# HerreraKrachTeichmann/NJODE

Measured on AMD Instinct MI355X. Metric: paths/sec (training step) on 20k Black-Scholes, 100 steps, higher is better.
Workload: dtype f32; 1 GPU; BlackScholes 20000 paths/GPU x 100 grid steps, every rank's paths as one batch, hidden_size=10, 3x(50,50) tanh nets, dropout 0.1, train step = plan+fwd+bwd+Adam; global_batch=20000, n_obs_rows=199470, euler_steps_per_batch=1820212, params=10071, parallelism=dp1

## Files before the change

include/njode_selftest.h:

```cpp
#ifndef NJODE_SELFTEST_H
#define NJODE_SELFTEST_H

#include <stdint.h>

#include "njode_hip.h"

#ifdef __cplusplus
extern "C" {
#endif

int njode_selftest_dropout_words(uint64_t seed, uint64_t path_id, uint32_t time_key, uint32_t net,
                                 int32_t n_words, uint32_t* out_words, void* stream);

int njode_debug_plan_stamps(unsigned long long* out, int cap_blocks);

typedef struct NjodePlanView {
  int64_t plan_bytes;
  int64_t sched;
  int64_t t_of_row, first_row, last_row;
  int64_t item_prev, item_next, item_kbeg, item_len;
  int64_t order, t_order;
  int64_t len_hist, base_s, base16_s, path_sorted, row_by_path, first_j;
  int64_t jlo, tile_base;
  int32_t n_tiles;
  int32_t generic;
  int32_t seg;
  int32_t sort_linked;
  int32_t links_only;
  int32_t tails;
  int32_t one_launch;
  int32_t plan_first_stage;
  int32_t plan_blocks;
  int32_t cs_shift, cs_nwb;
  int32_t cs_large;
  int32_t scan_thread_per_key;
  int32_t lds_cnt;
  int32_t tail_radix;
  int32_t split_on;
  int32_t split_ns[2], split_nw[2];
  float split_r[2];
} NjodePlanView;
int njode_debug_plan_view(const NjodeDims* dims, int32_t batch_size, int32_t n_obs, int32_t n_times,
                          int32_t n_steps, int32_t call_flags, NjodePlanView* out);

#ifdef __cplusplus
}
#endif
#endif
```

njode_amd/_lib.py:

```python
import ctypes as C
import os

import torch

_HERE = os.path.dirname(os.path.abspath(__file__))
LIB_PATH = os.environ.get('NJODE_LIB') or os.path.join(_HERE, 'libnjode_hip.so')

NJODE_OK = 0
E_UNSUPPORTED, E_BADARG, E_WORKSPACE, E_HIP = 1, 2, 3, 4
ACT_TANH, ACT_RELU = 0, 1
F_MASKED, F_INPUT_CURRENT_T, F_RESIDUAL, F_LOSS_EASY, F_USE_RNN = 0x1, 0x2, 0x4, 0x8, 0x10
C_TRAIN, C_GET_LOSS, C_RETURN_PATH, C_SAVE_BWD, C_LOSS_IN_BWD = 0x1, 0x2, 0x4, 0x8, 0x10
C_SCHED_KNOWN, C_SCHED_TAIL = 0x20, 0x40
C_PLAN_READY, C_NEED_HT = 0x80, 0x100
C_ROWS_IN_FWD = 0x400
C_GEN_LOCKSTEP = 0x200
C_PLAN_DEFER = 0x800

EXPORTS = ('njode_supported', 'njode_param_count', 'njode_workspace_bytes',
           'njode_plan_bytes', 'njode_plan_f32', 'njode_plan_flush', 'njode_plan_barrier_failures',
           'njode_forward_f32', 'njode_backward_f32', 'njode_backward_loss_f32',
           'njode_adam_step_f32',
           'njode_last_error', 'njode_build_info', 'njode_profile_enable',
           'njode_profile_read',
           'njode_philox4x32_10', 'njode_generate_paths', 'njode_sample_observations',
           'njode_collate_count', 'njode_collate_fill',
           'njode_cond_exp_bytes', 'njode_cond_exp_f64',
           'njode_generate_stage', 'njode_cond_exp_staged_bytes', 'njode_cond_exp_staged_f64',
           'njode_protocol_bytes', 'njode_protocol_rows', 'njode_protocol_score_f32',
           'njode_records_bytes', 'njode_records_count', 'njode_records_fill',
           'njode_records_heldout', 'njode_records_val_bytes', 'njode_records_val_count',
           'njode_records_val_fill',
           'njode_online_supported', 'njode_online_reset_f32', 'njode_online_advance_f32',
           'njode_online_observe_f32', 'njode_online_predict_f32', 'njode_online_run_f32',
           'njode_online_gen_supported', 'njode_online_tables_bytes', 'njode_online_tables_f32',
           'njode_online_gen_reset_f32', 'njode_online_gen_advance_f32', 'njode_online_gen_observe_f32',
           'njode_online_gen_predict_f32', 'njode_online_gen_run_f32',
           'njode_f64_supported', 'njode_f64_workspace_bytes', 'njode_forward_f64', 'njode_backward_f64',
           'njode_gob_supported', 'njode_gob_param_count', 'njode_gob_workspace_bytes',
           'njode_gob_forward_f32', 'njode_gob_backward_f32',
           'njode_selftest_dropout_words', 'njode_debug_plan_stamps', 'njode_debug_plan_view')
ROWS_CLOSEST, ROWS_FIRST_NEAREST = 0, 1
SDE_MODELS = {'BlackScholes': 0, 'OrnsteinUhlenbeck': 1, 'Heston': 2}
SDE_MODELS_STAGED = dict(SDE_MODELS, HestonWOFeller=3)
MAX_STAGES = 16


MAX_HIDDEN = 8


class NjodeNet(C.Structure):
    _fields_ = [('n_hidden', C.c_int32), ('width', C.c_int32 * MAX_HIDDEN),
                ('act', C.c_int32 * MAX_HIDDEN)]


class NjodeDims(C.Structure):
    _fields_ = [('input_size', C.c_int32), ('hidden_size', C.c_int32),
                ('output_size', C.c_int32), ('n_hidden', C.c_int32),
                ('width', C.c_int32), ('act', C.c_int32), ('flags', C.c_int32),
                ('per_net', C.c_int32), ('nets', NjodeNet * 3)]


class NjodeSchedule(C.Structure):
    _fields_ = [('n_steps', C.c_int32), ('n_times', C.c_int32),
                ('step_dt', C.c_void_p), ('step_t', C.c_void_p),
                ('k_jump', C.c_void_p), ('time_f32', C.c_void_p),
                ('time_ptr', C.c_void_p)]


class NjodeBatch(C.Structure):
    _fields_ = [('batch_size', C.c_int32), ('n_obs', C.c_int32),
                ('start_X', C.c_void_p), ('X', C.c_void_p), ('M', C.c_void_p),
                ('obs_idx', C.c_void_p), ('n_obs_ot', C.c_void_p),
                ('loss_batch_size', C.c_float), ('path_id_offset', C.c_int64),
                ('plan', C.c_void_p), ('grad_hT', C.c_void_p)]


class NjodeSchedule64(C.Structure):
    _fields_ = NjodeSchedule._fields_


class NjodeBatch64(C.Structure):
    _fields_ = [('batch_size', C.c_int32), ('n_obs', C.c_int32),
                ('start_X', C.c_void_p), ('X', C.c_void_p), ('M', C.c_void_p),
                ('obs_idx', C.c_void_p), ('n_obs_ot', C.c_void_p),
                ('loss_batch_size', C.c_double)]


GOB_F_BIAS, GOB_F_IMPUTE = 0x1, 0x2


class NjodeGobDims(C.Structure):
    _fields_ = [('input_size', C.c_int32), ('hidden_size', C.c_int32), ('p_hidden', C.c_int32),
                ('prep_hidden', C.c_int32), ('cov_hidden', C.c_int32), ('flags', C.c_int32)]


class NjodeSde(C.Structure):
    _fields_ = [('model', C.c_int32), ('n_paths', C.c_int32), ('dim', C.c_int32),
                ('n_steps', C.c_int32), ('has_sine', C.c_int32), ('reserved', C.c_int32),
                ('drift', C.c_double), ('volatility', C.c_double), ('mean', C.c_double),
                ('speed', C.c_double), ('correlation', C.c_double), ('S0', C.c_double),
                ('maturity', C.c_double), ('sine_coeff', C.c_double)]


class NjodeSdeStage(C.Structure):
    _fields_ = [('sde', NjodeSde), ('v0', C.c_double), ('return_vol', C.c_int32),
                ('first_step', C.c_int32)]


class NjodeCondExpSchedule(C.Structure):
    _fields_ = [('n_steps', C.c_int32), ('n_times', C.c_int32),
                ('step_dt', C.c_void_p), ('step_t', C.c_void_p),
                ('k_jump', C.c_void_p), ('time_ptr', C.c_void_p)]


class NjodeProtocolJob(C.Structure):
    _fields_ = [('pred', C.c_void_p), ('n_rows', C.c_int32), ('B', C.c_int32), ('dim', C.c_int32),
                ('n_query', C.c_int32), ('rows', C.c_void_p), ('vals', C.c_void_p),
                ('mask', C.c_void_p), ('X_val', C.c_void_p), ('M_val', C.c_void_p),
                ('index_val', C.c_void_p)]


class NjodeRecordStore(C.Structure):
    _fields_ = [('n_records', C.c_int32), ('n_rows', C.c_int32), ('dim', C.c_int32),
                ('n_grid', C.c_int32), ('drop_unobserved', C.c_int32), ('reserved', C.c_int32),
                ('row_ptr', C.c_void_p), ('row_g', C.c_void_p), ('vals', C.c_void_p),
                ('mask', C.c_void_p), ('att_min', C.c_void_p), ('att_max', C.c_void_p)]


class NjodeOnlineState(C.Structure):
    _fields_ = [('h', C.c_void_p), ('last_X', C.c_void_p), ('tau', C.c_void_p), ('now', C.c_void_p),
                ('n_series', C.c_int32)]


class NjodePlanView(C.Structure):
    OFFSETS = ('sched', 't_of_row', 'first_row', 'last_row', 'item_prev', 'item_next', 'item_kbeg',
               'item_len', 'order', 't_order', 'len_hist', 'base_s', 'base16_s', 'path_sorted',
               'row_by_path', 'first_j', 'jlo', 'tile_base')
    FLAGS = ('n_tiles', 'generic', 'seg', 'sort_linked', 'links_only', 'tails', 'one_launch',
             'plan_first_stage', 'plan_blocks', 'cs_shift', 'cs_nwb', 'cs_large', 'scan_thread_per_key', 'lds_cnt',
             'tail_radix', 'split_on')
    _fields_ = ([('plan_bytes', C.c_int64)] + [(n, C.c_int64) for n in OFFSETS]
                + [(n, C.c_int32) for n in FLAGS]
                + [('split_ns', C.c_int32 * 2), ('split_nw', C.c_int32 * 2), ('split_r', C.c_float * 2)])

    def as_dict(self):
        d = {n: int(getattr(self, n)) for n in ('plan_bytes',) + self.OFFSETS + self.FLAGS}
        d.update(split_ns=list(self.split_ns), split_nw=list(self.split_nw), split_r=list(self.split_r))
        return d


def plan_view(dims, batch_size, n_obs, n_times, n_steps, call_flags):
    v = NjodePlanView()
    check(lib().njode_debug_plan_view(C.byref(dims), batch_size, n_obs, n_times, n_steps, call_flags,
                                      C.byref(v)))
    return v.as_dict()


class NjodeError(RuntimeError):
    def __init__(self, code, msg):
        super().__init__('libnjode_hip error {}: {}'.format(code, msg))
        self.code = code


class NjodeUnsupported(NjodeError, NotImplementedError):
    pass


_lib = None


def lib():
    global _lib
    if _lib is not None:
        return _lib
    if not os.path.exists(LIB_PATH):
        raise ImportError(
            'njode_amd: {} not found. The NJ-ODE path has no CPU fallback; build '
            'the gfx950 library first: `python -m njode_amd.build` (needs hipcc).'
            .format(LIB_PATH))
    L = C.CDLL(LIB_PATH)
    vp, i32, f32, u64, sz = C.c_void_p, C.c_int32, C.c_float, C.c_uint64, C.c_size_t
    L.njode_supported.argtypes = [C.POINTER(NjodeDims)]
    L.njode_supported.restype = C.c_int
    L.njode_param_count.argtypes = [C.POINTER(NjodeDims)]
    L.njode_param_count.restype = sz
    L.njode_workspace_bytes.argtypes = [C.POINTER(NjodeDims), i32, i32, i32, i32, i32,
                                        C.POINTER(sz)]
    L.njode_workspace_bytes.restype = C.c_int
    L.njode_plan_bytes.argtypes = [C.POINTER(NjodeDims), i32, i32, i32, i32, i32, C.POINTER(sz)]
    L.njode_plan_bytes.restype = C.c_int
    L.njode_plan_f32.argtypes = [C.POINTER(NjodeDims), C.POINTER(NjodeBatch),
                                 C.POINTER(NjodeSchedule), i32, vp, sz, vp]
    L.njode_plan_f32.restype = C.c_int
# ... 150 lines not shown
```

njode_amd/csrc/njode_api.hip:

```cpp
#include <hip/hip_runtime.h>

#include <cmath>
#include <cstdio>
#include <cstring>

#include "../../include/njode_selftest.h"
#include "njode_call.h"
#include "njode_gen_host.h"
#include "njode_layout.h"

using namespace njode;

#define NJ_CFG(ID) namespace njode { const CfgOps* njode_cfg_ops_##ID(); }
#include "_generated_cfgs.inc"
#undef NJ_CFG
typedef const CfgOps* (*CfgGetter)();
static const CfgGetter g_cfgs[] = {
#define NJ_CFG(ID) njode::njode_cfg_ops_##ID,
#include "_generated_cfgs.inc"
#undef NJ_CFG
};
static const int g_ncfg = sizeof(g_cfgs) / sizeof(g_cfgs[0]);

static thread_local char g_err[512] = "";
// ... 249 lines not shown
  const size_t i = (size_t)blockIdx.x * blockDim.x + threadIdx.x;
  if (i >= n) return;
  const float pi = p[i];
  const float gi = fmaf(wd, pi, g[i] * gscale);
  const float mi = fmaf(beta1, m[i], (1.0f - beta1) * gi);
  const float vi = fmaf(beta2, v[i], (1.0f - beta2) * gi * gi);
  m[i] = mi;
  v[i] = vi;
  const float denom = sqrtf(vi) * inv_sqrt_c2 + eps;
  p[i] = pi - lr_c1 * (mi / denom);
}

TDesc transpose_desc(const CfgOps* o) {
  TDesc d;
  d.n = 0;
  const int nh = o->dims.n_hidden, W = o->dims.width, H = o->dims.hidden_size;
  const int ins[3] = {o->ode_in, o->enc_in, H};
  const int outs[3] = {H, H, o->dims.output_size};
  int off = 0;
  for (int net = 0; net < 3; ++net) {
    for (int l = 0; l <= nh; ++l) {
      const int li = l == 0 ? ins[net] : W, lo = l == nh ? outs[net] : W;
      d.l[d.n++] = {off, li, lo};
      off += li * lo + lo;
    }
  }
  if (o->dims.flags & NJODE_F_USE_RNN) {
    const int D = o->dims.input_size;
    d.l[d.n++] = {off, D, 3 * H};
    d.l[d.n++] = {off + 3 * H * D, H, 3 * H};
  }
  return d;
}

int prepare(Call& c, const NjodeDims* dims, const float* params, const NjodeBatch* b,
            const NjodeSchedule* s, int call_flags, float weight, float dropout_p,
            uint64_t seed, void* ws, size_t ws_bytes, bool want_hT, bool plan_only = false) {
  if (!dims || (!params && !plan_only) || !ws) return fail(NJODE_E_BADARG, "null argument");
  if (int rc = check_call(b, s, dims->flags, call_flags, dropout_p)) return rc;
  c.plan_only = plan_only;
  c.o = find_cfg(dims);
  if (!c.o)
    return fail(NJODE_E_UNSUPPORTED,
                "no gfx950 specialisation for d=%d H=%d d_out=%d n_hidden=%d width=%d act=%d "
                "flags=0x%x (compiled: %s)",
                dims->input_size, dims->hidden_size, dims->output_size, dims->n_hidden,
                dims->width, dims->act, dims->flags, njode_build_info());
  const int B = b->batch_size, n_obs = b->n_obs, K = s->n_steps, nt = s->n_times;
  const Sizing z = size_call(*c.o, B, n_obs, nt, K, call_flags, record_budget_bytes(), env());
  c.L = make_layout(c.o, z, B, n_obs, nt, K);
  if (ws_bytes < (plan_only ? c.L.plan_end : c.L.total))
    return fail(NJODE_E_WORKSPACE, "workspace too small: %zu < %zu", ws_bytes,
                plan_only ? c.L.plan_end : c.L.total);
  char* w = (char*)ws;
  c.planned = !plan_only && (call_flags & NJODE_C_PLAN_READY) != 0;
  if (c.planned && !b->plan) return fail(NJODE_E_BADARG, "NJODE_C_PLAN_READY without NjodeBatch.plan");
  char* pw = c.planned ? (char*)b->plan : w;
  c.pw = pw;
  KArgs& a = c.a;
  memset(&a, 0, sizeof(a));
  a.P = params;
  a.PT = (float*)(w + c.L.PT);
  a.frag = (float*)(w + c.L.frag);
  a.frag_enc = a.frag + c.o->frag_enc_off;
  a.frag_dec = a.frag + c.o->frag_dec_off;
  a.frag2 = a.frag + c.o->frag2_off;
  a.B = B;
  a.n_obs = n_obs;
  a.start_X = b->start_X;
  a.X = b->X;
  a.M = b->M;
  a.obs_idx = b->obs_idx;
  a.n_obs_ot = b->n_obs_ot;
  a.inv_batch = 1.0f / b->loss_batch_size;
  a.gid0 = (unsigned long long)b->path_id_offset;
  a.K = K;
  a.n_times = nt;
  float* sb = (float*)(pw + c.L.sched);
  a.step_dt = sb;
  a.step_t = sb + K;
  a.k_jump = (const int*)(sb + 2 * (size_t)K);
  a.time_f32 = sb + 2 * (size_t)K + nt;
  a.t_of_row = (int*)(pw + c.L.t_of_row);
  a.row_by_path = (int*)(pw + c.L.row_by_path);
  a.path_sorted = (int*)(pw + c.L.path_sorted);
  int* f3 = (int*)(pw + c.L.first3);
  a.first_j = f3;
  a.first_row = f3 + B;
  a.last_row = f3 + 2 * (size_t)B;
  int* i4 = (int*)(pw + c.L.item4);
  const size_t nr = (size_t)(n_obs > 0 ? n_obs : 1);
  a.item_prev = i4;
  a.item_next = i4 + nr;
  a.item_kbeg = i4 + 2 * nr;
  a.item_len = i4 + 3 * nr;
  a.order = (int*)(pw + c.L.order);
  a.t_order = (int*)(pw + c.L.tail4) + 3 * (size_t)B;
  a.base_s = (long long*)(pw + c.L.base_s);
  a.base16_s = (long long*)(pw + c.L.base16);
  a.act = c.L.act ? (float*)(w + c.L.act) : nullptr;
  a.dbits = c.L.dbits ? (uint32_t*)(w + c.L.dbits) : nullptr;
  a.dbits_row = c.L.dbits_row ? (uint32_t*)(w + c.L.dbits_row) : nullptr;
  a.q4_pt = z.q4_pt;
  a.chain = z.chain ? 1 : 0;
  a.h0row = (float*)(w + c.L.h0row);
  a.h0start = (float*)(w + c.L.h0start);
  a.h_end = (float*)(w + c.L.h_end);
  a.lam_end = (float*)(w + c.L.lam_end);
  a.g_h0 = (float*)(w + c.L.g_h0);
  a.lam_start = (float*)(w + c.L.lam_start);
  a.loss_terms = (float*)(w + c.L.loss_terms);
  a.traj = (float*)(w + c.L.traj);
  a.ltraj = a.traj;
  a.lam_traj = (float*)(w + c.L.lk_lam);
  a.src_row = (int*)(w + c.L.lk_src);
  float* rows = (float*)(w + c.L.lk_rows);
  const size_t nrDO = nr * dims->output_size;
  a.y_row = rows;
  a.ybj_row = rows + nrDO;
  a.g_y = rows + 2 * nrDO;
  a.g_ybj = rows + 3 * nrDO;
  a.g_hnew = rows + 4 * nrDO;
  a.g_hstart = (float*)(w + c.L.lk_hstart);
  a.lact = c.L.lk_act ? (float*)(w + c.L.lk_act) : nullptr;
  a.jact = c.L.lk_jact ? (float*)(w + c.L.lk_jact) : nullptr;
  a.cdelta = c.L.lk_delta ? (float*)(w + c.L.lk_delta) : nullptr;
  a.cseg = c.L.lk_seg ? (float*)(w + c.L.lk_seg) : nullptr;
  a.item_pack = c.L.item_pack ? (float*)(w + c.L.item_pack) : nullptr;
  a.tile_last = c.L.tile_last ? (long long*)(w + c.L.tile_last) : nullptr;
  a.slab = (float*)(w + c.L.slab);
  a.trash = (float*)(w + c.L.trash);
  a.g_hT = nullptr;
  a.n_waves = a.n_waves_ode = a.n_waves_rows = z.n_waves;
  a.weight = weight;
  a.loss_easy = (dims->flags & NJODE_F_LOSS_EASY) ? 1 : 0;
  const bool drop = (call_flags & NJODE_C_TRAIN) && dropout_p > 0.0f && dims->n_hidden > 0;
  if (drop && dims->width > 64)
    return fail(NJODE_E_UNSUPPORTED, "dropout needs width <= 64");
  const DropSetup ds = make_drop_ctx(dropout_p, seed, drop);
  a.dc = ds.dc;
  a.keep = ds.keep;
  const bool tail = (call_flags & NJODE_C_SCHED_KNOWN) ? (call_flags & NJODE_C_SCHED_TAIL) != 0
                                                        : (nt == 0 ? K > 0 : s->k_jump[nt - 1] < K);
  const Route& r = c.route = route_call(*c.o, z, B, n_obs, K, call_flags, env(), tail, drop, want_hT);
  if (!route_admitted(r))
    return fail(NJODE_E_WORKSPACE, "route not admitted by the workspace sizing (seg_chain %d / seg_items %d, "
                "lockstep kinds %d %d / chain %d lock_act %d, bits ahead %d %d / sized %d %d)",
                r.seg_chain, (int)z.seg_items, r.lock_fwd_kind, r.lock_bwd_kind, (int)z.chain, (int)z.lock_act,
                (int)r.seg_bits_ahead, (int)r.lock_bits_ahead, (int)z.seg_bits, (int)z.lock_bits);
  a.save_traj = z.save ? 1 : 0;
  a.ode_split = r.ode_split, a.seg_chain = r.seg_chain;
  a.defer_loss = r.defer_loss;
  a.n_split_blocks = r.n_split_blocks, a.n_blocks_bwd = r.n_blocks_bwd;
  a.n_split_fwd = r.n_split_fwd, a.n_blocks_fwd = r.n_blocks_fwd;
  a.dw_pair_blocks = r.dw_pair_blocks, a.dw_seg_blocks = r.dw_seg_blocks, a.dw_enc_fused = r.dw_enc_fused;
  return NJODE_OK;
}

__global__ void __launch_bounds__(1024) k_sum_small(const float* __restrict__ x, int n,
                                                    float* __restrict__ out) {
  __shared__ float sh[1024];
  float acc = 0.0f;
  for (int i = threadIdx.x; i < n; i += 1024) acc += x[i];
  sh[threadIdx.x] = acc;
  __syncthreads();
  for (int o = 512; o > 0; o >>= 1) {
    if ((int)threadIdx.x < o) sh[threadIdx.x] += sh[threadIdx.x + o];
    __syncthreads();
  }
  if (threadIdx.x == 0) out[0] = sh[0];
}
constexpr int SUM_SMALL_MAX = 16384;
void sum_to(const Call& c, void* ws, int n, float* out, hipStream_t st) {
  if (n <= SUM_SMALL_MAX) {
    k_sum_small<<<1, 1024, 0, st>>>(c.a.loss_terms, n, out);
    return;
  }
  float* partial = (float*)((char*)ws + c.L.sum_partial);
  k_sum_stage1<<<SUM_BLOCKS, 256, 0, st>>>(c.a.loss_terms, n, partial);
  k_sum_stage2<<<1, SUM_BLOCKS, 0, st>>>(partial, out);
}

int size_query(const NjodeDims* dims, int B, int n_obs, int n_times, int K, int call_flags, size_t* out, bool plan) {
  const CfgOps* o = find_cfg(dims);
  if (!o) return gen::gen_workspace_bytes(dims, B, n_obs, n_times, K, call_flags, out, plan);
  if (!out || B <= 0 || n_obs < 0 || n_times < 0 || K < 0) return fail(NJODE_E_BADARG, "bad size");
  const Layout L = make_layout(o, size_call(*o, B, n_obs, n_times, K, call_flags, record_budget_bytes(), env()),
                               B, n_obs, n_times, K);
  *out = plan ? L.plan_end : L.total;
  return NJODE_OK;
}

}

extern "C" int njode_workspace_bytes(const NjodeDims* dims, int32_t batch_size, int32_t n_obs,
                                     int32_t n_times, int32_t n_steps, int32_t call_flags, size_t* out) {
  return size_query(dims, batch_size, n_obs, n_times, n_steps, call_flags, out, false);
}

extern "C" int njode_plan_bytes(const NjodeDims* dims, int32_t batch_size, int32_t n_obs,
                                int32_t n_times, int32_t n_steps, int32_t call_flags, size_t* out) {
  return size_query(dims, batch_size, n_obs, n_times, n_steps, call_flags, out, true);
}

extern "C" int njode_debug_plan_view(const NjodeDims* dims, int32_t batch_size, int32_t n_obs, int32_t n_times,
                                     int32_t n_steps, int32_t call_flags, NjodePlanView* out) {
  if (!dims || !out) return fail(NJODE_E_BADARG, "null argument");
  memset(out, 0, sizeof(*out));
  out->sched = out->t_of_row = out->first_row = out->last_row = out->item_prev = out->item_next = out->item_kbeg =
      out->item_len = out->order = out->t_order = out->len_hist = out->base_s = out->base16_s = out->path_sorted =
          out->row_by_path = out->first_j = out->jlo = out->tile_base = -1;
  const int flags = call_flags & ~(NJODE_C_PLAN_READY | NJODE_C_PLAN_DEFER);
  size_t bytes = 0;
  if (int rc = size_query(dims, batch_size, n_obs, n_times, n_steps, flags, &bytes, true)) return rc;
  out->plan_bytes = (int64_t)bytes;
  if (!find_cfg(dims)) return gen::gen_plan_view(dims, batch_size, n_obs, n_times, n_steps, flags, out);
  alignas(256) static char anchor[256];
  NjodeBatch b{};
  b.batch_size = batch_size;
  b.n_obs = n_obs;
  b.start_X = b.X = b.M = (const float*)anchor;
  b.obs_idx = b.n_obs_ot = (const int32_t*)anchor;
  b.loss_batch_size = 1.0f;
  NjodeSchedule s{};
  s.n_steps = n_steps;
  s.n_times = n_times;
  s.step_dt = s.step_t = s.time_f32 = (const float*)anchor;
  s.k_jump = s.time_ptr = (const int32_t*)anchor;
  Call c;
  if (int rc = prepare(c, dims, nullptr, &b, &s, flags | NJODE_C_SCHED_KNOWN, 0.5f, 0.0f, 0, anchor, bytes,
                       (call_flags & NJODE_C_NEED_HT) != 0, true))
    return rc;
  const KArgs& a = c.a;
  const auto off = [&](const void* p) { return (int64_t)((const char*)p - anchor); };
  out->sched = off(a.step_dt);
  if (n_obs <= 0) return NJODE_OK;
  describe_plan(c, call_flags, out);
  out->t_of_row = off(a.t_of_row);
  out->first_row = off(a.first_row);
  out->last_row = off(a.last_row);
  out->item_prev = off(a.item_prev);
  out->item_next = off(a.item_next);
  out->item_kbeg = off(a.item_kbeg);
  out->item_len = off(a.item_len);
  out->len_hist = (int64_t)c.L.len_hist;
  if (out->sort_linked) {
    out->path_sorted = off(a.path_sorted);
    out->row_by_path = off(a.row_by_path);
    out->first_j = off(a.first_j);
  }
  if (out->seg && !out->links_only) {
    out->order = off(a.order);
    out->base_s = off(a.base_s);
    out->base16_s = off(a.base16_s);
  }
  if (out->tails) out->t_order = off(a.t_order);
  return NJODE_OK;
}

extern "C" int njode_plan_f32(const NjodeDims* dims, const NjodeBatch* batch,
                              const NjodeSchedule* sched, int32_t call_flags, void* plan,
                              size_t plan_bytes, njodeStream_t stream) {
  if (dims && !find_cfg(dims))
    return gen::gen_plan(dims, batch, sched, call_flags & ~(NJODE_C_PLAN_READY | NJODE_C_PLAN_DEFER), plan,
                         plan_bytes, (hipStream_t)stream);
  Call c;
  int rc = prepare(c, dims, nullptr, batch, sched, call_flags & ~(NJODE_C_PLAN_READY | NJODE_C_PLAN_DEFER), 0.5f,
                   0.0f, 0, plan, plan_bytes, (call_flags & NJODE_C_NEED_HT) != 0, true);
  if (rc) return rc;
  return plan_call(c, sched, call_flags, (hipStream_t)stream);
}

extern "C" int njode_forward_f32(const NjodeDims* dims, const float* params,
                                 const NjodeBatch* batch, const NjodeSchedule* sched,
                                 int32_t call_flags, float weight, float dropout_p,
                                 uint64_t seed, float* hT, float* loss, float* path_h,
                                 float* path_y, void* workspace, size_t workspace_bytes,
                                 njodeStream_t stream) {
  struct FlushGuard { ~FlushGuard() { pending_flush(); } } flush_on_any_return;
  if (dims && !find_cfg(dims)) {
    pending_flush();
    return gen::gen_forward(dims, params, batch, sched, call_flags, weight, dropout_p, seed, hT, loss,
                            path_h, path_y, workspace, workspace_bytes, (hipStream_t)stream);
  }
  Call c;
  int rc = prepare(c, dims, params, batch, sched, call_flags, weight, dropout_p, seed, workspace,
                   workspace_bytes, hT != nullptr);
  if (rc) return rc;
  const Route& r = c.route;
  hipStream_t st = (hipStream_t)stream;
  const bool want_loss = call_flags & NJODE_C_GET_LOSS, want_path = call_flags & NJODE_C_RETURN_PATH;
  if ((want_loss && !loss) || (want_path && (!path_h || !path_y)))
    return fail(NJODE_E_BADARG, "null output");
  if (!hT && !r.seg) return fail(NJODE_E_BADARG, "hT may only be omitted on the segment plan");
  if ((call_flags & NJODE_C_SAVE_BWD) && !(call_flags & NJODE_C_GET_LOSS))
    return fail(NJODE_E_BADARG, "NJODE_C_SAVE_BWD needs NJODE_C_GET_LOSS");
  c.a.hT = hT;
  c.a.path_h = path_h;
  c.a.path_y = path_y;
  if (c.planned) {
    if (r.tails && !(call_flags & NJODE_C_NEED_HT))
      return fail(NJODE_E_BADARG, "the prebuilt plan was made without NJODE_C_NEED_HT");
  } else {
    if ((rc = upload_schedule(c.pw + c.L.sched, sched, st))) return rc;
    if ((rc = build_plan(c, c.pw, st))) return rc;
  }
  PendingPlan hosted;
  pending_host_or_flush(c, st, hosted);
  if (r.seg) {
    route_side(c.route, c.a.plan_ready != nullptr);
    HIP_TRY(c.o->seg_forward(c.a, r, st));
    if (hosted.on) pending_tails(hosted);
    if (r.defer_loss != 1) sum_to(c, workspace, c.a.n_obs, loss, st);
  } else {
    HIP_TRY(c.o->lock_forward(c.a, r, st));
    if (want_loss) sum_to(c, workspace, c.a.B, loss, st);
  }
  HIP_TRY(hipGetLastError());
  return NJODE_OK;
}

static int backward_impl(const NjodeDims* dims, const float* params, const NjodeBatch* batch,
                         const NjodeSchedule* sched, int32_t call_flags, float weight,
                         float dropout_p, uint64_t seed, const float* grad_loss,
                         float* grad_params, float* loss, void* workspace,
                         size_t workspace_bytes, njodeStream_t stream) {
  if (dims && !find_cfg(dims))
    return gen::gen_backward(dims, params, batch, sched, call_flags, weight, dropout_p, seed,
                             grad_loss, grad_params, workspace, workspace_bytes, (hipStream_t)stream);
  Call c;
  int rc = prepare(c, dims, params, batch, sched, call_flags, weight, dropout_p, seed, workspace,
                   workspace_bytes, false);
  if (rc) return rc;
  const Route& r = c.route;
  if (!grad_loss || !grad_params) return fail(NJODE_E_BADARG, "null gradient pointer");
  if (!(call_flags & NJODE_C_SAVE_BWD) || !(call_flags & NJODE_C_GET_LOSS))
    return fail(NJODE_E_BADARG,
                "backward needs a forward with NJODE_C_SAVE_BWD | NJODE_C_GET_LOSS");
  hipStream_t st = (hipStream_t)stream;
  if (r.needs_PT) {
    const TDesc d = transpose_desc(c.o);
    k_transpose_params<<<cdiv(c.o->P, 256), 256, 0, st>>>(params, (float*)c.a.PT, c.o->P, d);
  }
  if (!r.seg && !r.lock_mfma && (dims->flags & NJODE_F_MASKED))
    return fail(NJODE_E_UNSUPPORTED,
                "the backward of a masked model runs on the matrix-core lockstep kernels only "
                "(2 hidden layers, width < 64, hidden_size <= 64, output_size <= 64)");
  if (r.lock_mfma) c.a.n_waves_rows = r.size.n_waves_lock;
  if (r.defer_loss == 1 && !loss)
    return fail(NJODE_E_BADARG, "NJODE_C_LOSS_IN_BWD needs njode_backward_loss_f32");
  if (batch->grad_hT && r.seg)
    return fail(NJODE_E_UNSUPPORTED, "NjodeBatch.grad_hT: the segment plan does not differentiate through hT; "
                                     "run the step with NJODE_C_GEN_LOCKSTEP");
  c.a.g_hT = batch->grad_hT;
  if (r.seg) HIP_TRY(c.o->seg_backward(c.a, r, st));
// ... 98 lines not shown
```

njode_amd/csrc/njode_cfg.hip:

```cpp
#include <type_traits>

#include "njode_route.h"
#if NJ_PART >= 4
#include "njode_chain.h"
#include "njode_chain_seg.h"
#include "njode_chain_dw.h"
#endif
#if NJ_PART == 6
#include "njode_online.h"
#endif

#define NJ_CAT_(a, b) a##b
#define NJ_CAT(a, b) NJ_CAT_(a, b)

namespace njode {

#ifndef NJ_RNN
#define NJ_RNN 0
#endif
using C = Cfg<NJ_D, NJ_H, NJ_DO, NJ_NH, NJ_W, NJ_ACT, (NJ_MASKED != 0), (NJ_CURT != 0),
              (NJ_RES != 0), (NJ_RNN != 0)>;

hipError_t NJ_CAT(njode_seg_forward_, NJ_ID)(const KArgs& a, const Route& r, hipStream_t st);
hipError_t NJ_CAT(njode_seg_backward_, NJ_ID)(const KArgs& a, const Route& r, hipStream_t st);
// ... 4 lines not shown
constexpr bool HAS_SPLIT = HAS_MFMA && SplitOk<C>::value;
constexpr bool HAS_Q4 = HAS_MFMA_SWEEP && Q4Ok<C>::value;
constexpr bool HAS_CHAIN = HAS_Q4 && ChainOk<C>::value;
void NJ_CAT(njode_chain_forward_, NJ_ID)(const KArgs& a, const Route& r, hipStream_t st);
void NJ_CAT(njode_chain_sweep_, NJ_ID)(const KArgs& a, const Route& r, hipStream_t st);
void NJ_CAT(njode_chain_dw_, NJ_ID)(const KArgs& a, hipStream_t st);
constexpr bool HAS_SEG_CHAIN = HAS_SPLIT && HAS_MFMA_SWEEP && SegChainOk<C>::value;
void NJ_CAT(njode_seg_chain_forward_, NJ_ID)(const KArgs& a, const Route& r, hipStream_t st);
void NJ_CAT(njode_seg_chain_backward_, NJ_ID)(const KArgs& a, const Route& r, hipStream_t st);

template <class F> static auto with_drop(bool drop, F f) {
  return drop ? f(std::true_type{}) : f(std::false_type{});
}
static inline const char* seg_fwd_name(const Route& r, bool tails) {
  if (r.seg_ode != ODE_MFMA) return tails ? "k_ode_fwd_items.tails" : "k_ode_fwd_items";
  if (r.seg_chain) return "k_seg_fwd_chain";
  if (r.ode_split) return tails ? "k_ode_fwd_split.tails" : "k_ode_fwd_mixed";
  return tails ? "k_ode_fwd_mfma.tails" : "k_ode_fwd_mfma";
}
static inline const char* lock_name(int kind, bool bwd) {
  if (kind == LOCK_VALU) return bwd ? "k_paths_bwd_adj" : "k_paths_fwd";
  if (kind == LOCK_CHAIN) return bwd ? "k_paths_bwd_adj_chain" : "k_paths_fwd_chain";
  return bwd ? "k_paths_bwd_adj_mfma" : "k_paths_fwd_mfma";
}
template <bool ON, class CC> struct FragSize {
  static constexpr int ode = 0, enc = 0, dec = 0;
};
template <class CC> struct FragSize<true, CC> {
  static constexpr int ode = MF<CC>::NALL * 64;
  static constexpr int enc = EncS<CC>::type::NALL * 64;
  static constexpr int dec = DecS<CC>::type::NALL * 64;
};
using FS = FragSize<(HAS_MFMA || HAS_MFMA_LOCK), C>;
constexpr int MF_FLOATS = FS::ode + FS::enc + FS::dec + FS::ode;
constexpr int FRAG2_OFF = FS::ode + FS::enc + FS::dec;
template <bool ON, class CC> struct ActSize { static constexpr int value = 0; };
template <class CC> struct ActSize<true, CC> { static constexpr int value = StepRec<CC>::PER_CHAIN; };
constexpr int ACT_FLOATS = ActSize<HAS_SPLIT, C>::value;

template <class C, class ES, class DS>
__global__ void k_pack_all(const float* __restrict__ P, float* __restrict__ frag, float* __restrict__ frag2,
                           float* __restrict__ frag_enc, float* __restrict__ frag_dec, float ik,
                           unsigned* __restrict__ zero8) {
  constexpr int N = MF<C>::NALL * 64, NE = ES::NALL * 64, ND = DS::NALL * 64;
  const int idx = blockIdx.x * blockDim.x + threadIdx.x;
  if (zero8 && idx < 8) zero8[idx] = 0;
  if (idx < N) frag[idx] = ode_frag_value<C>(P, idx, 1.0f, 1.0f);
  else if (idx < 2 * N) frag2[idx - N] = ode_frag_value<C>(P, idx - N, Ode2Scale<C>::S, ik);
  else if (idx < 2 * N + NE) pack_net_value<typename C::Enc, ES>(P + C::OFF_ENC, frag_enc, idx - 2 * N);
  else if (idx < 2 * N + NE + ND) pack_net_value<typename C::Dec, DS>(P + C::OFF_DEC, frag_dec, idx - 2 * N - NE);
}
template <class C, class ES, class DS>
__global__ void k_pack_all_bits(KArgs a, int n_pack) {
  if ((int)blockIdx.x < n_pack) {
    constexpr int N = MF<C>::NALL * 64, NE = ES::NALL * 64, ND = DS::NALL * 64;
    const int idx = blockIdx.x * blockDim.x + threadIdx.x;
    if (a.plan_sync_zero && idx < 8) a.plan_sync_zero[idx] = 0;
    if (idx < N) a.frag[idx] = ode_frag_value<C>(a.P, idx, 1.0f, 1.0f);
    else if (idx < 2 * N) a.frag2[idx - N] = ode_frag_value<C>(a.P, idx - N, Ode2Scale<C>::S, a.dc.inv_keep);
    else if (idx < 2 * N + NE) pack_net_value<typename C::Enc, ES>(a.P + C::OFF_ENC, a.frag_enc, idx - 2 * N);
    else if (idx < 2 * N + NE + ND) pack_net_value<typename C::Dec, DS>(a.P + C::OFF_DEC, a.frag_dec, idx - 2 * N - NE);
  } else {
    if constexpr (SegChainOk<C>::value) {
      if (a.seg_chain) {
        seg_chain_bits_body<C>(a, (int)blockIdx.x - n_pack, (int)gridDim.x - n_pack);
        return;
      }
    }
    if constexpr (HAS_SPLIT) {
      const int nb = (int)gridDim.x - n_pack;
      drop_bits_tile_steps<C>(a, ((int)blockIdx.x - n_pack) * 4 + (threadIdx.x >> 6), nb * 4);
    }
  }
}

template <class CC> static void launch_pack_frags(const KArgs& a, hipStream_t st, bool bits = false) {
  if constexpr (HAS_MFMA) {
    using ES = typename EncS<CC>::type;
    using DS = typename DecS<CC>::type;
    const int n_pack = cdiv((2 * MF<CC>::NALL + ES::NALL + DS::NALL) * 64, 256);
    if (bits) {
      const long long work = a.seg_chain ? (long long)a.K * a.B / 64 + 1
                                         : (long long)cdiv(a.n_obs, 16) * cdiv(a.K > 0 ? a.K : 1, 8);
      const int nb = (int)(work / 4 + 1 < 1024 ? work / 4 + 1 : 1024);
      k_pack_all_bits<CC, ES, DS><<<n_pack + nb, 256, 0, st>>>(a, n_pack);
    } else {
      k_pack_all<CC, ES, DS><<<n_pack, 256, 0, st>>>(a.P, a.frag, a.frag2, a.frag_enc, a.frag_dec, a.dc.inv_keep,
                                                  a.plan_sync_zero);
    }
  }
}
template <class CC, bool DROP> static void launch_mfma_enc(const KArgs& a, const Route& r, hipStream_t st) {
  if constexpr (HAS_MFMA) {
    const int n_tiles = cdiv(a.n_obs + a.B, 16);
    k_encode_rows_mfma<CC, DROP><<<n_tiles < r.enc_blocks ? n_tiles : r.enc_blocks, 64, 0, st>>>(a);
  }
}
template <class CC> static void lock_pack_frags(const KArgs& a, hipStream_t st) {
  if constexpr (HAS_MFMA_LOCK) {
    using ES = typename EncS<CC>::type;
    using DS = typename DecS<CC>::type;
    k_pack_frags<CC><<<cdiv(MF<CC>::NALL * 64, 256), 256, 0, st>>>(a.P, a.frag);
    k_pack_net<typename CC::Enc, ES><<<cdiv(ES::NALL * 64, 256), 256, 0, st>>>(a.P + CC::OFF_ENC,
                                                                             a.frag_enc);
    k_pack_net<typename CC::Dec, DS><<<cdiv(DS::NALL * 64, 256), 256, 0, st>>>(a.P + CC::OFF_DEC,
                                                                             a.frag_dec);
  }
}
template <class CC, bool DROP> static void launch_mfma_jump(const KArgs& a, hipStream_t st) {
  if constexpr (HAS_MFMA) {
    const int n_tiles = cdiv(a.n_obs, 16);
    k_jump_rows_mfma<CC, DROP><<<n_tiles < 2048 ? n_tiles : 2048, 64, 0, st>>>(a);
  }
}
template <class CC, bool DROP> static void launch_ode_bwd_mfma(const KArgs& a, const Route& r, hipStream_t st) {
  if constexpr (HAS_MFMA) {
    if constexpr (HAS_SPLIT) {
      if (r.ode_split) {
        ProfScope ps("k_ode_bwd_mixed", st);
        k_ode_bwd_mixed<CC, DROP><<<a.n_blocks_bwd, 256, 0, st>>>(a);
        return;
      }
    }
    ProfScope ps("k_ode_bwd_mfma", st);
    k_ode_bwd_mfma<CC, DROP><<<a.n_waves_ode / 4, 256, 0, st>>>(a);
  }
}
template <class CC, bool DROP> static void launch_jump_rows_bwd(const KArgs& a, hipStream_t st) {
  if constexpr (HAS_MFMA) {
    ProfScope ps("k_jump_rows_bwd_mfma", st);
    k_jump_rows_bwd_mfma<CC, DROP><<<a.n_waves_rows / 4, 256, 0, st>>>(a);
  }
}
template <class CC, bool DROP>
static void launch_mfma_rows_bwd(const KArgs& a, const Route& r, hipStream_t st) {
  if constexpr (HAS_MFMA) {
    if (r.defer_loss != 2) launch_jump_rows_bwd<CC, DROP>(a, st);
    if (r.seg_chain) NJ_CAT(njode_seg_chain_backward_, NJ_ID)(a, r, st);
    else launch_ode_bwd_mfma<CC, DROP>(a, r, st);
    if (!r.dw_enc_fused) {
      ProfScope ps("k_encode_rows_bwd_mfma", st);
      k_encode_rows_bwd_mfma<CC, DROP><<<a.n_waves_rows / 4, 256, 0, st>>>(a);
    }
  }
}
template <class CC, bool DROP, bool TAIL>
static void launch_mfma_fwd(const KArgs& a, const Route& r, hipStream_t st) {
  if constexpr (HAS_MFMA) {
    const int n_tiles = cdiv(TAIL ? a.B : a.n_obs, 16);
    if constexpr (HAS_SPLIT) {
      if (r.ode_split) {
        if constexpr (TAIL) {
          k_ode_fwd_split<CC, DROP, true><<<n_tiles < 1024 ? n_tiles : 1024, 256, 0, st>>>(a);
        }
        else if (a.plan_job) {
          const PlanJob job = *(const PlanJob*)a.plan_job;
          k_ode_fwd_mixed_plan<CC, DROP><<<a.n_blocks_fwd + job.P, 256, 0, st>>>(a, job);
        }
        else k_ode_fwd_mixed<CC, DROP><<<a.n_blocks_fwd, 256, 0, st>>>(a);
        return;
      }
    }
    k_ode_fwd_mfma<CC, DROP, TAIL><<<n_tiles < 4096 ? n_tiles : 4096, 64, 0, st>>>(a);
  }
}

hipError_t NJ_CAT(njode_lock_forward_, NJ_ID)(const KArgs& a, const Route& r, hipStream_t st);
hipError_t NJ_CAT(njode_lock_backward_, NJ_ID)(const KArgs& a, const Route& r, hipStream_t st);

#if NJ_PART == 0
template <bool DROP, bool TAIL, int ODE> static void launch_ode_fwd(const KArgs& a, const Route& r, hipStream_t st) {
  const int n_items = TAIL ? a.B : a.n_obs;
  if constexpr (ODE == ODE_MFMA) {
    launch_mfma_fwd<C, DROP, TAIL>(a, r, st);
  } else {
    k_ode_fwd_items<C, DROP, TAIL><<<cdiv(n_items, 64), 64, 0, st>>>(a);
  }
}
template <bool DROP, int ODE>
static hipError_t seg_forward_t(const KArgs& a, const Route& r, hipStream_t st) {
  if constexpr (C::MASKED || C::RNN) {
    return hipErrorNotSupported;
  } else {
    const SideInfo* side = r.side ? (const SideInfo*)a.plan_ready : nullptr;
    hipStream_t s2 = side ? side->st : st;
    if (side) (void)hipStreamWaitEvent(s2, side->e0, 0);
    KArgs ab = a;
    if constexpr (ODE == ODE_MFMA) {
      ab.dbits_ready = r.seg_bits_ahead ? 1 : 0;
      if (ab.plan_sync_zero && s2 != st) {
        (void)hipMemsetAsync(ab.plan_sync_zero, 0, 8 * sizeof(unsigned), st);
        ab.plan_sync_zero = nullptr;
      }
      ProfScope ps("k_pack_all", s2);
      launch_pack_frags<C>(ab, s2, r.seg_bits_ahead);
    }
    {
      ProfScope ps(ODE == ODE_MFMA ? "k_encode_rows_mfma" : "k_encode_rows", s2);
      if constexpr (ODE == ODE_MFMA) launch_mfma_enc<C, DROP>(a, r, s2);
      else k_encode_rows<C, DROP><<<cdiv(a.n_obs + a.B, 64), 64, 0, s2>>>(a);
    }
    if (side) {
      (void)hipEventRecord(side->e1, s2);
      (void)hipStreamWaitEvent(st, side->e1, 0);
    }
    if (r.tails_side) {
      (void)hipStreamWaitEvent(side->st2, side->e1, 0);
      if (!side->tails_sorted_on_st2) {
        (void)hipEventRecord(side->e0, st);
        (void)hipStreamWaitEvent(side->st2, side->e0, 0);
      }
    }
    {
      ProfScope ps(seg_fwd_name(r, false), st);
      if (r.seg_chain) NJ_CAT(njode_seg_chain_forward_, NJ_ID)(ab, r, st);
      else launch_ode_fwd<DROP, false, ODE>(ab, r, st);
    }
    if (r.tails_side) {
      ProfScope ps(seg_fwd_name(r, true), side->st2);
      launch_ode_fwd<DROP, true, ODE>(a, r, side->st2);
      (void)hipEventRecord(side->e2, side->st2);
    } else if (r.tails && !r.tails_ride) {
      ProfScope ps(seg_fwd_name(r, true), st);
      launch_ode_fwd<DROP, true, ODE>(a, r, st);
    }
    if (r.defer_loss == 2) {
      launch_jump_rows_bwd<C, DROP>(a, st);
    } else if (!r.defer_loss) {
      ProfScope ps(ODE == ODE_MFMA ? "k_jump_rows_mfma" : "k_jump_rows", st);
      if constexpr (ODE == ODE_MFMA) launch_mfma_jump<C, DROP>(a, st);
      else k_jump_rows<C, DROP><<<cdiv(a.n_obs, 64), 64, 0, st>>>(a);
    }
    if (r.tails_side) (void)hipStreamWaitEvent(st, side->e2, 0);
    return hipGetLastError();
  }
}
hipError_t NJ_CAT(njode_seg_forward_, NJ_ID)(const KArgs& a, const Route& r, hipStream_t st) {
  return with_drop(r.drop, [&](auto D) {
    constexpr bool DROP = decltype(D)::value;
    return r.seg_ode == ODE_MFMA ? seg_forward_t<DROP, ODE_MFMA>(a, r, st) : seg_forward_t<DROP, ODE_VALU>(a, r, st);
  });
}

const CfgOps* NJ_CAT(njode_cfg_ops_, NJ_ID)() {
  static const CfgOps ops = {
      {NJ_D, NJ_H, NJ_DO, NJ_NH, (NJ_NH > 0 ? NJ_W : 0), NJ_ACT,
       (NJ_MASKED ? NJODE_F_MASKED : 0) | (NJ_CURT ? NJODE_F_INPUT_CURRENT_T : 0) |
           (NJ_RES ? NJODE_F_RESIDUAL : 0) | (NJ_RNN ? NJODE_F_USE_RNN : 0)},
      C::P,
      C::ODE_IN,
      C::ENC_IN,
      C::OFF_ENC,
      C::OFF_DEC,
      NJ_CAT(njode_seg_forward_, NJ_ID),
      NJ_CAT(njode_seg_backward_, NJ_ID),
      NJ_CAT(njode_lock_forward_, NJ_ID),
      NJ_CAT(njode_lock_backward_, NJ_ID),
      MF_FLOATS,
      FS::ode,
      FS::ode + FS::enc,
      FRAG2_OFF,
      ACT_FLOATS,
      HAS_Q4 ? Q4_ACT_FLOATS : 0,
      HAS_MFMA_LOCK ? 1 : 0,
      HAS_MFMA_SWEEP ? 1 : 0,
      HAS_CHAIN ? 1 : 0,
      HAS_SEG_CHAIN ? 1 : 0,
      HAS_SPLIT ? 1 : 0,
      HAS_MFMA ? 1 : 0};
  return &ops;
}
#endif

#if NJ_PART == 1
template <bool DROP, int ODE> static hipError_t seg_backward_t(const KArgs& a, const Route& r, hipStream_t st) {
  if constexpr (C::MASKED || C::RNN) {
    return hipErrorNotSupported;
  } else if constexpr (ODE == ODE_MFMA) {
    launch_mfma_rows_bwd<C, DROP>(a, r, st);
    return hipGetLastError();
  } else {
    {
      ProfScope ps("k_jump_rows_bwd", st);
      k_jump_rows_bwd<C, DROP><<<a.n_waves, 64, 0, st>>>(a);
    }
    {
      ProfScope ps("k_ode_bwd_items", st);
      k_ode_bwd_items<C, DROP><<<a.n_waves, 64, 0, st>>>(a);
    }
    {
      ProfScope ps("k_encode_rows_bwd", st);
      k_encode_rows_bwd<C, DROP><<<a.n_waves, 64, 0, st>>>(a);
    }
    return hipGetLastError();
  }
}
hipError_t NJ_CAT(njode_seg_backward_, NJ_ID)(const KArgs& a, const Route& r, hipStream_t st) {
  return with_drop(r.drop, [&](auto D) {
    constexpr bool DROP = decltype(D)::value;
    return r.seg_ode == ODE_MFMA ? seg_backward_t<DROP, ODE_MFMA>(a, r, st) : seg_backward_t<DROP, ODE_VALU>(a, r, st);
  });
}
#endif

#if NJ_PART == 2
template <class CC, bool DROP> static void lock_launch_mfma(const KArgs& a, const Route& r, hipStream_t st) {
  if (r.lock_fwd_kind == LOCK_CHAIN) {
    NJ_CAT(njode_chain_forward_, NJ_ID)(a, r, st);
  } else if (r.lock_fwd_kind == LOCK_TILE4) {
    if constexpr (HAS_Q4) {
      const int n_tiles = cdiv(a.B, a.q4_pt);
      KArgs ab = a;
// ... 216 lines not shown
```

njode_amd/csrc/njode_env.h:

```cpp
#pragma once
#include <cstdlib>
#include <cstring>

namespace njode {

constexpr int ODE_MFMA = 0, ODE_VALU = 1;

struct Env {
  bool lock4, drop_bits_ahead, generic, ode_one_wave, sort_merge, sort_rocprim, item_pack, chain_delta, lock_sweep_valu,
      dw_enc_fused, tail_sort_rocprim, validate, plan_sort, plan_grid, plan_stamps, plan_stream, plan_grid_tail;
  int lock4_pt, chain_max, seg_chain_max, ode, split_bwd_blocks, split_fwd_blocks, bwd_blocks, fwd_blocks,
      plan_blocks, cs_shift, plan_inline_max, plan_inline_blocks, enc_blocks, chain_wpb,
      gen_nw, gen_pt, gen_dbg;
  float split_r_bwd, split_r_fwd;
  double rec_budget_gb;
};

inline Env parse_env() {
  const auto num = [](const char* name, int dflt) { const char* e = getenv(name); return e ? atoi(e) : dflt; };
  const auto real = [](const char* name, double dflt) { const char* e = getenv(name); return e ? atof(e) : dflt; };
  const auto on = [](const char* name) { const char* e = getenv(name); return e && atoi(e) != 0; };
  const auto not_off = [](const char* name) { const char* e = getenv(name); return !(e && atoi(e) == 0); };
  const auto is = [](const char* e, const char* v) { return e && strcmp(e, v) == 0; };
  const char *ode = getenv("NJODE_ODE"), *sort = getenv("NJODE_SORT"), *lock4 = getenv("NJODE_LOCK4");
  Env e;
  e.lock4 = !(lock4 && lock4[0] == '0');
  e.drop_bits_ahead = not_off("NJODE_DROP_BITS_AHEAD");
  e.enc_blocks = num("NJODE_ENC_BLOCKS", 4096);
  e.chain_wpb = num("NJODE_CHAIN_WPB", 0);
  e.generic = on("NJODE_GENERIC");
  e.rec_budget_gb = real("NJODE_REC_BUDGET_GB", 16.0);
  e.lock4_pt = num("NJODE_LOCK4_PT", 0);
  e.chain_max = num("NJODE_CHAIN_MAX", 1 << 30);
  e.seg_chain_max = num("NJODE_SEG_CHAIN_MAX", 16384);
  e.ode = is(ode, "valu") ? ODE_VALU : ODE_MFMA;
  e.ode_one_wave = is(ode, "mfma1");
  e.sort_merge = is(sort, "merge");
  e.sort_rocprim = is(sort, "rocprim");
  e.item_pack = not_off("NJODE_ITEM_PACK");
  e.chain_delta = not_off("NJODE_CHAIN_DELTA");
  e.split_r_bwd = (float)real("NJODE_SPLIT_R_BWD", 2.25);
  e.split_r_fwd = (float)real("NJODE_SPLIT_R_FWD", 2.0);
  e.lock_sweep_valu = is(getenv("NJODE_LOCK_SWEEP"), "valu");
  e.split_bwd_blocks = num("NJODE_SPLIT_BWD_BLOCKS", 32);
  e.split_fwd_blocks = num("NJODE_SPLIT_FWD_BLOCKS", 96);
  e.bwd_blocks = num("NJODE_BWD_BLOCKS", 0);
  e.fwd_blocks = num("NJODE_FWD_BLOCKS", 3072);
  e.dw_enc_fused = not_off("NJODE_DW_ENC_FUSED");
  e.tail_sort_rocprim = is(getenv("NJODE_TAIL_SORT"), "rocprim");
  e.plan_blocks = num("NJODE_PLAN_BLOCKS", 0);
  e.validate = on("NJODE_VALIDATE");
  e.plan_sort = is(getenv("NJODE_PLAN"), "sort");
  e.plan_grid = not_off("NJODE_PLAN_GRID");
  e.cs_shift = num("NJODE_CS_SHIFT", 8);
  e.plan_stamps = on("NJODE_PLAN_STAMPS");
  e.plan_inline_max = num("NJODE_PLAN_INLINE_MAX", 16384);
  e.plan_stream = not_off("NJODE_PLAN_STREAM");
  e.plan_grid_tail = not_off("NJODE_PLAN_GRID_TAIL");
  e.plan_inline_blocks = num("NJODE_PLAN_INLINE_BLOCKS", 128);
  e.gen_nw = num("NJODE_GEN_NW", -1);
  e.gen_pt = num("NJODE_GEN_PT", 0);
  e.gen_dbg = num("NJODE_GEN_DBG", 0);
  return e;
}
inline const Env& env() {
  static const Env e = parse_env();
  return e;
}

}
```

njode_amd/csrc/njode_kernels.h:

```cpp
#pragma once
#include "njode_device.h"

namespace njode {

constexpr uint32_t NET_ODE = 0, NET_ENC = 1, NET_DEC = 2, NET_DEC_BJ = 3, NET_DEC_ROW = 4;
constexpr uint32_t TKEY_START = 0xffffffffu;

template <int D_, int H_, int DO_, int NH_, int W_, int ACT_, bool MASKED_, bool CURT_,
          bool RES_, bool RNN_ = false>
struct Cfg {
  static constexpr int D = D_, H = H_, DO = DO_, NH = NH_, W = (NH_ > 0 ? W_ : 1), ACT = ACT_;
  static constexpr bool MASKED = MASKED_, CURT = CURT_, RES = RES_, RNN = RNN_;
  static constexpr int ODE_IN = D + H + (CURT ? 3 : 2);
  static constexpr int ENC_IN = MASKED ? 2 * D : D;
  using Ode = NetL<ODE_IN, H, NH, W_>;
  using Enc = NetL<ENC_IN, H, NH, W_>;
  using Dec = NetL<H, DO, NH, W_>;
  static constexpr int OFF_ODE = 0, OFF_ENC = Ode::SIZE, OFF_DEC = Ode::SIZE + Enc::SIZE;
  static constexpr int OFF_GRU = OFF_DEC + Dec::SIZE;
  static constexpr int G_WIH = 0, G_WHH = 3 * H * D, G_BIH = G_WHH + 3 * H * H, G_BHH = G_BIH + 3 * H;
  static constexpr int GRU_SIZE = G_BHH + 3 * H;
  static constexpr int P = OFF_GRU + (RNN ? GRU_SIZE : 0);
  static_assert(!(RNN && MASKED), "the GRU jump is not defined for masked models");
  static constexpr int ENC_CASE = !RES ? 0 : (D <= H ? 1 : 2);
  static constexpr int DEC_CASE = !RES ? 0 : (H <= DO ? 1 : 2);
  static_assert(!RES || (D <= H ? H % D == 0 : D % H == 0), "residual: sizes must divide");
  static_assert(!RES || (H <= DO ? DO % H == 0 : H % DO == 0), "residual: sizes must divide");
  static_assert(!MASKED || D == DO, "masked mode imputes X with the readout");
};

struct KArgs {
  const float* P;
  const float* PT;
  float* frag;
  float* frag_enc;
  float* frag_dec;
  float* frag2;
  const void* fragx;
  void* plan_ready;
  const void* plan_job;
  int B, n_obs;
  const float* start_X;
  const float* X;
  const float* M;
  const int* obs_idx;
  const int* n_obs_ot;
  float inv_batch;
  unsigned long long gid0;
  int K, n_times;
  const float* step_dt;
  const float* step_t;
  const int* k_jump;
  const float* time_f32;
  const int* t_of_row;
  const int* row_by_path;
  const int* path_sorted;
  const int* first_j;
  const int* first_row;
  const int* last_row;
  const int* item_prev;
  const int* item_next;
  const int* item_kbeg;
  const int* item_len;
  const int* order;
  const int* t_order;
  const long long* base_s;
  const long long* base16_s;
  float* act;
  uint32_t* dbits;
  int dbits_ready;
  uint32_t* dbits_row;
  float* h0row;
  float* h0start;
  float* h_end;
  float* lam_end;
  float* g_h0;
  float* lam_start;
  float* traj;
  float* ltraj;
  float* lam_traj;
  int* src_row;
  float* y_row;
  float* ybj_row;
  float* g_y;
  float* g_ybj;
  float* g_hnew;
  float* g_hstart;
  float* lact;
  float* jact;
  float* loss_terms;
  float* slab;
  float* trash;
  unsigned* plan_sync_zero;
  int args_pad;
  int n_waves;
  int n_waves_ode;
  int n_waves_rows;
  const float* g_hT;
  float* hT;
  float* path_h;
  float* path_y;
  float weight;
  int loss_easy;
  int want_path, want_loss;
  int save_traj;
  int defer_loss;
  int ode_split;
  int n_split_blocks, n_blocks_bwd, n_split_fwd, n_blocks_fwd;
  int q4_pt;
  int chain;
  int seg_chain;
  float* cdelta;
  float* cseg;
  float* item_pack;
  long long* tile_last;
  int dw_pair_blocks, dw_seg_blocks;
  int dw_enc_fused;
  DropCtx dc;
  float keep;
};

template <class C, bool TWO = (C::NH == 2)> struct ChainOk { static constexpr bool value = false; };
template <class C> struct ChainOk<C, true> {
  static constexpr bool value =
      C::MASKED && !C::RNN && C::W <= 64 && C::H <= 64 && C::D <= 64 && C::DO <= 64 && C::D == C::DO &&
      (C::ENC_CASE == 0 || (C::ENC_CASE == 1 && C::D == C::H)) &&
      (C::DEC_CASE == 0 || (C::DEC_CASE == 1 && C::DO == C::H));
};
template <class C, bool TWO = (C::NH == 2)> struct SegChainOk { static constexpr bool value = false; };
template <class C> struct SegChainOk<C, true> {
  static constexpr bool value = !C::MASKED && !C::RNN && C::W <= 64 && C::W > 16 && C::H <= 16 && C::D <= 8;
};
constexpr int CHAIN_MAX_WAVES = 8;
constexpr int CHAIN_ACT_FLOATS = 2 * 64;
constexpr int CHAIN_JACT_FLOATS = 3 * 2 * 64;

template <int N> NJ_DEV void load_vec(const float* p, float (&v)[N]) {
#pragma unroll
  for (int i = 0; i < N; ++i) v[i] = p[i];
}
template <int N> NJ_DEV void store_vec(float* p, const float (&v)[N]) {
#pragma unroll
  for (int i = 0; i < N; ++i) p[i] = v[i];
}
NJ_DEV int wave_max(int v) {
#pragma unroll
  for (int o = 32; o > 0; o >>= 1) v = max(v, __shfl_xor(v, o));
  return v;
}

template <class C, bool DROP> struct Masks {
  uint64_t m1 = 0, m2 = 0;
  NJ_DEV void draw(const KArgs& a, unsigned long long gid, uint32_t tkey, uint32_t net) {
    if constexpr (DROP && C::NH > 0) {
      uint32_t s = drop_state(a.dc, (uint32_t)gid, (uint32_t)(gid >> 32), tkey, net);
      m1 = keep_mask<C::W>(s, a.dc.thr16);
      if constexpr (C::NH > 1) m2 = keep_mask<C::W>(s, a.dc.thr16);
    }
  }
};

template <class C, bool DROP, class WP>
NJ_DEV void encode(WP Pe, const float (&x)[C::D], const float (&mask)[C::D],
                   float (&ein)[C::ENC_IN], float (&a1)[C::W], float (&a2)[C::W],
                   const Masks<C, DROP>& mk, float inv_keep, float (&h)[C::H]) {
#pragma unroll
  for (int i = 0; i < C::D; ++i) ein[i] = tanh_f(x[i]);
  if constexpr (C::MASKED) {
#pragma unroll
    for (int i = 0; i < C::D; ++i) ein[C::D + i] = mask[i];
  }
  net_fwd<typename C::Enc, C::ACT, DROP>(Pe, ein, h, a1, a2, mk.m1, mk.m2, inv_keep);
  if constexpr (C::ENC_CASE == 1) {
#pragma unroll
    for (int j = 0; j < C::H; ++j) h[j] += x[j % C::D];
  } else if constexpr (C::ENC_CASE == 2) {
    constexpr int mult = C::D / C::H;
#pragma unroll
    for (int j = 0; j < C::H; ++j) {
      float s = 0.0f;
#pragma unroll
      for (int c = 0; c < mult; ++c) s += x[c * C::H + j];
      h[j] += s * (1.0f / mult);
    }
  }
}

template <class C, bool DROP, class WP>
NJ_DEV void readout(WP Pd, const float (&h)[C::H], float (&th)[C::H], float (&a1)[C::W],
                    float (&a2)[C::W], const Masks<C, DROP>& mk, float inv_keep,
                    float (&y)[C::DO]) {
#pragma unroll
  for (int i = 0; i < C::H; ++i) th[i] = tanh_f(h[i]);
  net_fwd<typename C::Dec, C::ACT, DROP>(Pd, th, y, a1, a2, mk.m1, mk.m2, inv_keep);
  if constexpr (C::DEC_CASE == 1) {
#pragma unroll
    for (int j = 0; j < C::DO; ++j) y[j] += h[j % C::H];
  } else if constexpr (C::DEC_CASE == 2) {
    constexpr int mult = C::H / C::DO;
#pragma unroll
    for (int j = 0; j < C::DO; ++j) {
      float s = 0.0f;
#pragma unroll
      for (int c = 0; c < mult; ++c) s += h[c * C::DO + j];
      y[j] += s * (1.0f / mult);
    }
  }
}

NJ_DEV float sigmoid_f(float x) {
  return __builtin_amdgcn_rcpf(1.0f + __builtin_amdgcn_exp2f(-1.4426950408889634f * x));
}
template <class C>
NJ_DEV void gru_jump(cfp Pg, const float (&x)[C::D], const float (&h)[C::H], float (&tx)[C::D],
                     float (&th)[C::H], float (&r)[C::H], float (&z)[C::H], float (&n)[C::H],
                     float (&ghn)[C::H], float (&hn)[C::H]) {
  constexpr int H = C::H, D = C::D;
  float gi[3 * H], gh[3 * H];
#pragma unroll
  for (int i = 0; i < D; ++i) tx[i] = tanh_f(x[i]);
#pragma unroll
  for (int i = 0; i < H; ++i) th[i] = tanh_f(h[i]);
  const cfp P = launder(Pg);
  dense<D, 3 * H>(P + C::G_WIH, P + C::G_BIH, tx, gi);
  dense<H, 3 * H>(P + C::G_WHH, P + C::G_BHH, th, gh);
#pragma unroll
  for (int i = 0; i < H; ++i) {
    r[i] = sigmoid_f(gi[i] + gh[i]);
    z[i] = sigmoid_f(gi[H + i] + gh[H + i]);
    ghn[i] = gh[2 * H + i];
    n[i] = tanh_f(gi[2 * H + i] + r[i] * ghn[i]);
    hn[i] = (1.0f - z[i]) * n[i] + z[i] * th[i];
  }
  pin(hn);
}

template <class C>
NJ_DEV void ode_input(const float (&tx)[C::D], const float (&h)[C::H], float tau, float t,
                      float (&in0)[C::ODE_IN]) {
#pragma unroll
  for (int i = 0; i < C::D; ++i) in0[i] = tx[i];
#pragma unroll
  for (int i = 0; i < C::H; ++i) in0[C::D + i] = tanh_f(h[i]);
  const float tdiff = t - tau;
  in0[C::D + C::H] = tau;
  in0[C::D + C::H + 1] = tdiff;
  if constexpr (C::CURT) in0[C::D + C::H + 2] = tau + tdiff;
}

template <class C>
NJ_DEV float loss_row(const float (&x)[C::D], const float (&mask)[C::D], const float (&y)[C::DO],
                      const float (&ybj)[C::DO], float w, int easy, float scale,
                      float (&dy)[C::DO], float (&dybj)[C::DO]) {
  static_assert(C::D == C::DO, "loss compares X with the readout");
  float sa = 0.0f, sb = 0.0f;
#pragma unroll
  for (int q = 0; q < C::D; ++q) {
    const float m = C::MASKED ? mask[q] : 1.0f;
    const float e = x[q] - y[q];
    const float f = easy ? (ybj[q] - x[q]) : (ybj[q] - y[q]);
    sa = fmaf(m * e, e, sa);
    sb = fmaf(m * f, f, sb);
  }
  const float na = sqrtf(sa + 1e-10f), nb = sqrtf(sb + 1e-10f);
  const float ca = easy ? w : 2.0f * w, cb = easy ? (1.0f - w) : 2.0f * (1.0f - w);
  const float s = ca * na + cb * nb;
  const float g = 2.0f * s * scale;
  const float ga = g * ca / na, gb = g * cb / nb;
// ... 445 lines not shown
```

njode_amd/csrc/njode_layout.h:

```cpp
#pragma once
#include "njode_hostlib.h"
#include "njode_plan.h"
#include "njode_planner.h"
#include "njode_route.h"

namespace njode {

constexpr int SUM_BLOCKS = 64;
constexpr int RED_SPLIT = 32;

constexpr int PLAN_CS_SMALL_BLOCKS = 32;
struct Layout : Arena {
  size_t len_hist = 0, dense = 0;
  size_t sched, PT, frag, trash, t_of_row, iota, path_sorted, row_by_path, first3, item4, sort_key,
      key_sorted, order, tail4, base_s, h0row, h0start, h_end, lam_end, g_h0, lam_start, loss_terms,
      traj, slab, red_partial, sum_partial, sort_tmp, lk_lam, lk_src, lk_rows, lk_hstart, base16, act, dbits, dbits_row, lk_act, lk_jact, lk_delta, lk_seg, item_pack, tile_last, vflag, cs_small, plan_end;
  size_t sort_tmp_bytes = 0;
};

inline Layout make_layout(const CfgOps* o, const Sizing& z, int B, int n_obs, int n_times, int K) {
  Layout L{};
  const int H = o->dims.hidden_size, D = o->dims.input_size, DO = o->dims.output_size;
  const size_t nr = (size_t)(n_obs > 0 ? n_obs : 1), nb = (size_t)(B > 0 ? B : 1);
  const size_t steps = (size_t)(K > 0 ? K : 1);
  const int mx = H > D ? (H > DO ? H : DO) : (D > DO ? D : DO);
  L.sched = L.take(((size_t)2 * K + 3 * (size_t)n_times + 1) * 4 + 64);
  L.t_of_row = L.take(nr * 4);
  L.iota = L.take(nr * 4);
  L.path_sorted = L.take(nr * 4);
  L.row_by_path = L.take(nr * 4);
  L.first3 = L.take(nb * 4 * 3);
  L.item4 = L.take(nr * 4 * 4);
  L.sort_key = L.take(nr * 4);
  L.key_sorted = L.take(nr * 4);
  L.order = L.take(nr * 4);
  L.tail4 = L.take(nb * 4 * 4);
  L.base_s = L.take(((size_t)K + 4) * 8);
  L.base16 = L.take(((size_t)K + 2) * 8);
  L.len_hist = L.take(((size_t)K + 2) * 4);
  L.dense = L.take((z.dense_cells ? z.dense_cells : 1) * 4);
  L.sort_tmp_bytes = plan_sort_temp_bytes(n_obs, B, K);
  L.sort_tmp = L.take(L.sort_tmp_bytes);
  L.vflag = L.take(256);
  L.cs_small = L.take((size_t)PLAN_KEYS * PLAN_CS_SMALL_BLOCKS * 4);
  L.plan_end = L.total;
  L.PT = L.take((size_t)o->P * 4);
  L.frag = L.take((size_t)(o->frag_floats > 0 ? o->frag_floats : 1) * 4);
  L.trash = L.take((size_t)(256 * mx > 4096 ? 256 * mx : 4096) * 4);
  if (z.seg_bits) L.dbits = L.take(((size_t)B * K / 16 + (size_t)K + 2) * 256);
  L.h0row = L.take(nr * H * 4);
  L.h0start = L.take(nb * H * 4);
  L.h_end = L.take(nr * H * 4);
  L.lam_end = L.take(nr * H * 4);
  L.g_h0 = L.take(nr * H * 4);
  L.lam_start = L.take(nr * H * 4);
  L.loss_terms = L.take((nr > nb ? nr : nb) * 4);
  L.sum_partial = L.take(SUM_BLOCKS * 4);
  if (z.chain && z.lock_bits) {
    L.dbits = L.take(((size_t)B * steps + 1) * 16);
    L.dbits_row = L.take((nr * 3 + nb) * 16);
  }
  if (!z.save) return L;
  L.traj = L.take(((size_t)B * (K + 1) + 1) * H * 4);
  L.lk_lam = L.take(((size_t)B * K + 1) * H * 4);
  L.lk_src = L.take(((size_t)B * K + 1) * 4);
  L.lk_rows = L.take(nr * (size_t)(4 * DO + H) * 4);
  L.lk_hstart = L.take(nb * H * 4);
  L.slab = L.take((size_t)z.slab_rows * o->P * 4);
  L.red_partial = L.take((size_t)RED_SPLIT * o->P * 4);
  const size_t act_fl = z.seg_items && CHAIN_ACT_FLOATS > o->act_floats ? CHAIN_ACT_FLOATS : o->act_floats;
  if (z.seg_act) L.act = L.take(((size_t)B * K + 16 * ((size_t)K + 1)) * act_fl * 4);
  if (z.pack) {
    const size_t packf = 4 + 4 * (size_t)((1 + D + 3) / 4);
    L.item_pack = L.take((size_t)cdiv((int)nr, 16) * 16 * packf * 4);
    L.tile_last = L.take((size_t)cdiv((int)nr, 16) * 8);
  }
  if (z.chain) {
    L.lk_act = L.take((size_t)B * steps * CHAIN_ACT_FLOATS * 4);
    L.lk_jact = L.take(nr * (size_t)CHAIN_JACT_FLOATS * 4);
  } else if (z.lock_act) {
    static_assert(Q4_JACT_FLOATS == 3 * 2 * 4 * 4, "jump-activation record: 3 evaluations x 2 layers x 4 registers x 4 lane groups");
    L.lk_act = L.take((size_t)cdiv(B, z.q4_pt) * steps * o->lock_act_floats * 4);
    L.lk_jact = L.take(nr * 4 * (size_t)Q4_JACT_FLOATS * 4);
    if (z.lock_bits) {
      L.dbits = L.take((size_t)cdiv(B, z.q4_pt) * steps * 256);
      L.dbits_row = L.take(nr * 3 * 4 * 4);
    }
  }
  if (z.delta) L.lk_delta = L.take((size_t)B * steps * CHAIN_ACT_FLOATS * 4);
  if (z.delta_seg) L.lk_seg = L.take((nr + nb) * (size_t)CHAIN_ACT_FLOATS * 4);
  return L;
}

struct Call {
  const CfgOps* o;
  Route route;
  Layout L;
  KArgs a;
  SideInfo side;
  char* pw;
  bool planned;
  bool plan_only;
};

}
```

njode_amd/csrc/njode_mfma_split.h:

```cpp
#pragma once
#include "njode_mfma.h"
#include "njode_ode2.h"
#include "njode_plan.h"

namespace njode {

template <class C, bool TWO = (C::NH == 2)> struct SplitOk { static constexpr bool value = false; };
template <class C> struct SplitOk<C, true> {
  static constexpr bool value = MF<C>::MT1 == 4 && MF<C>::MTH == 1 && !C::MASKED && !C::RNN;
};

constexpr int XROWS = 64;
constexpr int XFLOATS = XROWS * IMG_STRIDE;
constexpr int TROWS = 16;
constexpr int TFLOATS = TROWS * IMG_STRIDE;

template <class C, bool BWD> struct SplitFrags {
  using M = MF<C>;
  float A1[M::Q0], A2[M::Q1], A3[4];
  float B3[BWD ? M::QH : 1], B2[BWD ? M::QW : 1], B1[BWD ? 4 : 1];
  NJ_DEV void load(const float* frag, int w, int lane) {
#pragma unroll
    for (int q = 0; q < M::Q0; ++q) A1[q] = frag[(M::F1 + w * M::Q0 + q) * 64 + lane];
#pragma unroll
    for (int q = 0; q < M::Q1; ++q) A2[q] = frag[(M::F2 + w * M::Q1 + q) * 64 + lane];
#pragma unroll
    for (int r = 0; r < 4; ++r) {
      const int q = 4 * w + r;
      A3[r] = q < M::Q1 ? frag[(M::F3 + (q < M::Q1 ? q : 0)) * 64 + lane] : 0.0f;
    }
    if constexpr (BWD) {
#pragma unroll
      for (int q = 0; q < M::QH; ++q) B3[q] = frag[(M::B3 + w * M::QH + q) * 64 + lane];
#pragma unroll
      for (int q = 0; q < M::QW; ++q) B2[q] = frag[(M::B2 + w * M::QW + q) * 64 + lane];
#pragma unroll
      for (int r = 0; r < 4; ++r) {
        const int q = 4 * w + r;
        B1[r] = q < M::QW ? frag[(M::B1 + (q < M::QW ? q : 0)) * 64 + lane] : 0.0f;
      }
    }
  }
};

NJ_DEV void block_lds_barrier() {
  asm volatile("s_waitcnt lgkmcnt(0)\n\ts_barrier" ::: "memory");
}

template <class C, bool DROP>
NJ_DEV void split_keep_bits(const KArgs& a, int b, int k, int g, int w, uint32_t& k1, uint32_t& k2) {
  constexpr int NWD = (MF<C>::Q1 + 1) / 2;
  k1 = k2 = 0;
  if constexpr (DROP) {
    const unsigned long long gid = a.gid0 + b;
    uint32_t st = drop_state(a.dc, (uint32_t)gid, (uint32_t)(gid >> 32) + 0x5bd1e995u * (g + 1),
                             (uint32_t)k, NET_ODE);
    auto skip = [&](int n) {
      for (int i = 0; i < n; ++i) { st ^= st << 13; st ^= st >> 17; st ^= st << 5; }
    };
    skip(2 * w);
    k1 = keep_bits<4>(st, a.dc.thr16);
    skip(NWD - 2);
    k2 = keep_bits<4>(st, a.dc.thr16);
  }
}

template <class C>
NJ_DEV void drop_bits_tile_steps(const KArgs& a, int worker, int n_workers) {
  using M = MF<C>;
  constexpr int CH = 8;
  const int lane = threadIdx.x & 63, g = lane >> 4, c = lane & 15;
  const int T = (int)a.base_s[a.K + 2];
  const int n_ch = (a.K + CH - 1) / CH;
  const long long n_work = (long long)T * n_ch;
  for (long long i = worker; i < n_work; i += n_workers) {
    const int tile = (int)(i / n_ch), s0 = (int)(i % n_ch) * CH;
    const int j = tile * 16 + c;
    const bool valid = j < a.n_obs;
    const int r = a.order[valid ? j : 0];
    const int n = valid ? a.item_len[r] : 0;
    const int nmax = uniform(wave_max(n));
    if (s0 >= nmax) continue;
    const int b = a.obs_idx[r], kbeg = a.item_kbeg[r];
    const unsigned long long gid = a.gid0 + b;
    for (int s = s0; s < s0 + CH && s < nmax; ++s) {
      const int k = s < n ? kbeg + s : 0;
      uint32_t st = drop_state(a.dc, (uint32_t)gid, (uint32_t)(gid >> 32) + 0x5bd1e995u * (g + 1),
                               (uint32_t)k, NET_ODE);
      const uint32_t k1 = keep_bits<M::Q1>(st, a.dc.thr16);
      const uint32_t k2 = keep_bits<M::Q1>(st, a.dc.thr16);
      a.dbits[(size_t)(sload_ll(a.base16_s, s) / 16 + tile) * 64 + lane] = k1 | (k2 << 16);
    }
  }
}

template <class C, bool DROP>
NJ_DEV void split_hidden(const f32x4& acc, float (&al)[4], float (&au)[4], uint32_t keep, float inv_keep,
                         int g, int w) {
#pragma unroll
  for (int r = 0; r < 4; ++r) {
    float v = act_f<C::ACT>(acc[r]), u = v;
    if constexpr (DROP) {
      const bool k = (keep >> r) & 1;
      u = k ? v : -0.0f;
      v = k ? v * inv_keep : 0.0f;
    }
    al[r] = v;
    au[r] = u;
  }
  constexpr int QB = C::W / 4, GB = C::W % 4;
  if (w == QB / 4) {
    al[QB % 4] = g == GB ? 1.0f : al[QB % 4];
    au[QB % 4] = g == GB ? 1.0f : au[QB % 4];
  }
}
template <class C, bool DROP>
NJ_DEV void split_delta(const f32x4& acc, const float (&al)[4], float (&dl)[4], uint32_t keep,
                        float inv_keep, float keepf, int g, int w) {
#pragma unroll
  for (int r = 0; r < 4; ++r) {
    const float gsum = acc[r];
    float d;
    if constexpr (DROP) d = ((keep >> r) & 1) ? gsum * inv_keep * dact_f<C::ACT>(al[r] * keepf) : 0.0f;
    else d = gsum * dact_f<C::ACT>(al[r]);
    dl[r] = (16 * w + 4 * r + g) < C::W ? d : 0.0f;
  }
}

NJ_DEV void split_put(lfp X, const float (&v)[4], int g, int c, int w) {
#pragma unroll
  for (int r = 0; r < 4; ++r) X[(16 * w + 4 * r + g) * IMG_STRIDE + c] = v[r];
}
template <int NQ> NJ_DEV void split_get(lfp X, float (&v)[NQ], int g, int c) {
#pragma unroll
  for (int q = 0; q < NQ; ++q) v[q] = X[(4 * q + g) * IMG_STRIDE + c];
}

template <class C>
NJ_DEV void split_rec_store(float* blk, float* trash, int lane, int w, const float (&a1u)[4],
                            const float (&a2u)[4], const float (&h)[MF<C>::QH]) {
  using R = StepRec<C>;
  float* bq = w < R::NF ? blk : trash;
  quad_store(bq + w * 256 + lane * 4, a2u[0], a2u[1], a2u[2], a2u[3]);
  quad_store(bq + R::GA + w * 256 + lane * 4, a1u[0], a1u[1], a1u[2], a1u[3]);
  float a2x[MF<C>::Q1];
#pragma unroll
  for (int q = 0; q < MF<C>::Q1; ++q) a2x[q] = 0.0f;
#pragma unroll
  for (int i = 0; i < R::L1; ++i) a2x[4 * R::NF + i] = a2u[i];
  rec_tail_store<C>(w == R::WT ? blk : trash, lane, a2x, h);
  if constexpr (R::L1 > 0) {
    float* bs = w == R::NF ? blk : trash;
#pragma unroll
    for (int i = 0; i < R::L1; ++i) bs[R::B1S + i * 64 + lane] = a1u[i];
  }
}
// ... 225 lines not shown
      }
      dtt = act ? a.step_dt[kk] : 0.0f;
      tt = a.step_t[kk];
    };
    float h_n[M::QH], dt_n = 0.0f, t_n = 0.0f;
#pragma unroll
    for (int q = 0; q < M::QH; ++q) h_n[q] = 0.0f;
    if (nmax > 0) fetch(nmax - 1, h_n, dt_n, t_n);
    for (int s = nmax - 1; s >= 0; --s) {
      const bool active = s < it.n;
      const int k = active ? it.kbeg + s : 0;
      float h[M::QH];
#pragma unroll
      for (int q = 0; q < M::QH; ++q) h[q] = h_n[q];
      const float dt = dt_n, t = t_n;
      if (s > 0) fetch(s - 1, h_n, dt_n, t_n);
      float b0[M::Q0], a1l[4], a2l[4];
      in0_fill<C, 0>(b0, h, it.tx, it.tau, t - it.tau, g);
      uint32_t k1, k2;
      split_keep_bits<C, DROP>(a, it.b, k, g, w, k1, k2);
      float a1u_[4], a2u_[4];
      split_hidden_layers<C, DROP, true>(F, X1, b0, a1l, a2l, a1u_, a2u_, k1, k2, a.dc.inv_keep, g, c, w);

      float d3[M::QH];
#pragma unroll
      for (int q = 0; q < M::QH; ++q) d3[q] = dt * lam[q];
      img_write<M::QH>(imgD3, d3, g, c);
#pragma unroll
      for (int r = 0; r < 4; ++r) imgA2[(4 * r + g) * IMG_STRIDE + c] = a2l[r];
      img_write<M::Q0>(imgB0, b0, g, c);
      f32x4 acc = z;
#pragma unroll
      for (int q = 0; q < M::QH; ++q) acc = mfma4(F.B3[q], d3[q], acc);
      float d2l[4], d1l[4];
      split_delta<C, DROP>(acc, a2l, d2l, k2, a.dc.inv_keep, a.keep, g, w);
      split_put(X2, d2l, g, c, w);
      wave_lds_sync();
      dw_accumulate<1, 1>(imgD3, imgA2, G3, g, c);
      block_lds_barrier();

      float d2[M::QW];
      split_get<M::QW>(X2, d2, g, c);
      __builtin_amdgcn_sched_barrier(0);
      f32x4 acc0 = z, acc1 = z;
#pragma unroll
      for (int q = 0; q < M::QW; q += 2) {
        acc0 = mfma4(F.B2[q], d2[q], acc0);
        if (q + 1 < M::QW) acc1 = mfma4(F.B2[q + 1], d2[q + 1], acc1);
      }
      dw_accumulate<1, NT1>(X2 + 16 * w * IMG_STRIDE, X1, G2, g, c);
      acc = acc0 + acc1;
      split_delta<C, DROP>(acc, a1l, d1l, k1, a.dc.inv_keep, a.keep, g, w);

#pragma unroll
      for (int r = 0; r < 4; ++r) imgD1[(4 * r + g) * IMG_STRIDE + c] = d1l[r];
      f32x4 part = z;
#pragma unroll
      for (int r = 0; r < 4; ++r)
        if (4 * w + r < M::QW) part = mfma4(F.B1[r], d1l[r], part);
      wave_lds_sync();
      dw_accumulate<1, 1>(imgD1, imgB0, G1, g, c);
      float gh[M::QH];
      split_reduce<M::QH>(PR, part, gh, lane, w);
#pragma unroll
      for (int q = 0; q < M::QH; ++q) {
        const float th = b0[q];
        const float dth = (4 * q + g) < C::H ? 1.0f - th * th : 0.0f;
        lam[q] = fmaf(gh[q], dth, lam[q]);
      }
    }
    if (w == 0) {
      float* out = valid ? a.lam_start + (size_t)it.r * C::H : trash;
#pragma unroll
      for (int q = 0; q < M::QH; ++q) {
        const int u = 4 * q + g;
        float* dst = u < C::H ? out + u : trash;
        *dst = lam[q];
      }
    }
  }

  float* slab = a.slab + (size_t)slab_row * C::P + C::OFF_ODE;
  float *W1 = slab + NL::woff(0), *b1 = slab + NL::boff(0), *W2 = slab + NL::woff(1),
        *b2 = slab + NL::boff(1), *W3 = slab + NL::woff(2), *b3 = slab + NL::boff(2);
#pragma unroll
  for (int r = 0; r < 4; ++r) {
    const int uo = 16 * w + 4 * g + r;
    if (uo < M::W) {
#pragma unroll
      for (int nt = 0; nt < NT1; ++nt) {
        const int ui = 16 * nt + c;
        if (ui < M::W) W2[uo * M::W + ui] = G2[0][nt][r];
        else if (ui == M::W) b2[uo] = G2[0][nt][r];
      }
      if (c < M::IN0) W1[uo * M::IN0 + M::col0(c)] = G1[0][0][r];
      else if (c == M::IN0) b1[uo] = G1[0][0][r];
    }
    const int uh = 4 * g + r, ui = 16 * w + c;
    if (uh < C::H) {
      if (ui < M::W) W3[uh * M::W + ui] = G3[0][0][r];
      else if (ui == M::W) b3[uh] = G3[0][0][r];
    }
  }
}


template <class C, bool DROP>
NJ_DEV void split_delta_stored(const f32x4& acc, const float (&au)[4], float (&dl)[4], float ik, int g, int w) {
#pragma unroll
  for (int r = 0; r < 4; ++r) {
    const float d = acc[r] * ik * dact_stored<C::ACT, DROP>(au[r]);
    dl[r] = (16 * w + 4 * r + g) < C::W ? d : 0.0f;
  }
}
template <class C> struct SplitFragsT {
  using M = MF<C>;
  float B3[M::QH], B2[M::QW], B1[4];
  NJ_DEV void load(const float* frag, int w, int lane) {
#pragma unroll
    for (int q = 0; q < M::QH; ++q) B3[q] = frag[(M::B3 + w * M::QH + q) * 64 + lane];
#pragma unroll
    for (int q = 0; q < M::QW; ++q) B2[q] = frag[(M::B2 + w * M::QW + q) * 64 + lane];
#pragma unroll
    for (int r = 0; r < 4; ++r) {
      const int q = 4 * w + r;
      B1[r] = q < M::QW ? frag[(M::B1 + (q < M::QW ? q : 0)) * 64 + lane] : 0.0f;
    }
  }
};

template <class C, bool DROP>
NJ_DEV void ode3_bwd_split(const KArgs& a, lfp lds_raw, int worker, int n_workers, int tile0, int tile1,
                          int slab_row) {
  using M = MF<C>;
  using NL = typename C::Ode;
  constexpr int NT1 = 4;
  static_assert((M::W + 1 + 15) / 16 == NT1 && (M::IN0 + 1 + 15) / 16 == 1,
                "split kernels: 4 column tiles of [a, 1], one of [in0, 1]");
  lfp X1 = lds_raw, X2 = X1 + XFLOATS, PR = X2 + XFLOATS;
  const int lane = threadIdx.x & 63, g = lane >> 4, c = lane & 15;
  const int w = __builtin_amdgcn_readfirstlane(threadIdx.x >> 6);
  lfp imgD3 = PR + 4 * M::QH * 64 + w * 4 * TFLOATS, imgA2 = imgD3 + TFLOATS, imgD1 = imgA2 + TFLOATS,
      imgB0 = imgD1 + TFLOATS;
  for (int i = threadIdx.x; i < 2 * XFLOATS + 4 * M::QH * 64 + 4 * 4 * TFLOATS; i += 256) lds_raw[i] = 0.0f;
  SplitFragsT<C> F;
  F.load(a.frag, w, lane);
  In0Const<C> K0;
  K0.init(g);
  __syncthreads();

  const f32x4 z = {0.f, 0.f, 0.f, 0.f};
  f32x4 G3[1][1] = {{z}}, G2[1][NT1] = {{z, z, z, z}}, G1[1][1] = {{z}};
  float* const trash = a.trash + lane * C::H;
  const int n_tiles = tile1 - tile0;
  BWD_STAMP(1, wall_clock64());
  int n_done = 0, n_steps_done = 0;
  for (int round = 0; round * n_workers < n_tiles; ++round) {
    const int rel = snake_tile(round, worker, n_workers);
    if (rel >= n_tiles) continue;
    const int tile = tile0 + rel;
    const int j = tile * 16 + c;
    const bool valid = j < a.n_obs;
    Item<C> it;
    it.template load<false>(a, j, valid);
    float lam[M::QH];
#pragma unroll
    for (int q = 0; q < M::QH; ++q) {
      const int u = 4 * q + g;
      const float v = a.lam_end[(size_t)it.r * C::H + (u < C::H ? u : 0)];
      lam[q] = (valid && u < C::H) ? v : 0.0f;
    }
    const int nmax = uniform(wave_max(it.n));
    ++n_done;
    n_steps_done += nmax;
    SplitRecRaw<C> nx;
    nx.zero();
    float dt_r = 0.0f, t_r = 0.0f;
    auto fetch = [&](int s) {
      const int kk = s < it.n ? it.kbeg + s : 0;
      nx.load(rec_block<C>(a.act, sload_ll(a.base16_s, s), tile), lane, w);
      dt_r = a.step_dt[kk];
      t_r = a.step_t[kk];
    };
    if (nmax > 0) fetch(nmax - 1);
    vm_drain();
    for (int s = nmax - 1; s >= 0; --s) {
      float h[M::QH], a1u[4], a2u[4];
      nx.unpack(w, a1u, a2u, h);
      const float dt = s < it.n ? dt_r : 0.0f, t = t_r;
      fetch(s > 0 ? s - 1 : 0);
      float b0[M::Q0], a1l[4], a2l[4];
      in0_fill_c<C, 0>(b0, h, it.tx, it.tau, t - it.tau, g, K0);
      const float ik = DROP ? a.dc.inv_keep : 1.0f;
#pragma unroll
      for (int r = 0; r < 4; ++r) { a1l[r] = a1u[r] * ik; a2l[r] = a2u[r] * ik; }
      constexpr int QBb = C::W / 4, GBb = C::W % 4;
      if (w == QBb / 4) {
        a1l[QBb % 4] = g == GBb ? 1.0f : a1l[QBb % 4];
        a2l[QBb % 4] = g == GBb ? 1.0f : a2l[QBb % 4];
      }
      split_put(X1, a1l, g, c, w);

      float d3[M::QH];
#pragma unroll
      for (int q = 0; q < M::QH; ++q) d3[q] = dt * lam[q];
      f32x4 acc = z;
#pragma unroll
      for (int q = 0; q < M::QH; ++q) acc = mfma4(F.B3[q], d3[q], acc);
      img_write<M::QH>(imgD3, d3, g, c);
#pragma unroll
      for (int r = 0; r < 4; ++r) imgA2[(4 * r + g) * IMG_STRIDE + c] = a2l[r];
      img_write<M::Q0>(imgB0, b0, g, c);
      float d2l[4], d1l[4];
      split_delta_stored<C, DROP>(acc, a2u, d2l, ik, g, w);
      split_put(X2, d2l, g, c, w);
      block_lds_barrier();

      float d2[M::QW];
      split_get<M::QW>(X2, d2, g, c);
      __builtin_amdgcn_sched_barrier(0);
      dw_accumulate<1, 1>(imgD3, imgA2, G3, g, c);
      f32x4 acc0 = z, acc1 = z;
#pragma unroll
      for (int q = 0; q < M::QW; q += 2) {
        acc0 = mfma4(F.B2[q], d2[q], acc0);
        if (q + 1 < M::QW) acc1 = mfma4(F.B2[q + 1], d2[q + 1], acc1);
      }
      dw_accumulate<1, NT1>(X2 + 16 * w * IMG_STRIDE, X1, G2, g, c);
      acc = acc0 + acc1;
      split_delta_stored<C, DROP>(acc, a1u, d1l, ik, g, w);

#pragma unroll
      for (int r = 0; r < 4; ++r) imgD1[(4 * r + g) * IMG_STRIDE + c] = d1l[r];
      f32x4 part = z;
#pragma unroll
      for (int r = 0; r < 4; ++r)
        if (4 * w + r < M::QW) part = mfma4(F.B1[r], d1l[r], part);
      wave_lds_sync();
      dw_accumulate<1, 1>(imgD1, imgB0, G1, g, c);
      float gh[M::QH];
      split_reduce<M::QH>(PR, part, gh, lane, w);
#pragma unroll
      for (int q = 0; q < M::QH; ++q) {
        const float th = b0[q];
        const float dth = (4 * q + g) < C::H ? 1.0f - th * th : 0.0f;
        lam[q] = fmaf(gh[q], dth, lam[q]);
      }
    }
    if (w == 0) {
      float* out = valid ? a.lam_start + (size_t)it.r * C::H : trash;
#pragma unroll
      for (int q = 0; q < M::QH; ++q) {
        const int u = 4 * q + g;
        float* dst = u < C::H ? out + u : trash;
        *dst = lam[q];
      }
    }
  }

  BWD_STAMP(2, wall_clock64());
  BWD_STAMP(4, (unsigned long long)n_done);
  BWD_STAMP(5, (unsigned long long)n_steps_done);
  (void)n_done; (void)n_steps_done;
  float* slab = a.slab + (size_t)slab_row * C::P + C::OFF_ODE;
  float *W1 = slab + NL::woff(0), *b1 = slab + NL::boff(0), *W2 = slab + NL::woff(1),
        *b2 = slab + NL::boff(1), *W3 = slab + NL::woff(2), *b3 = slab + NL::boff(2);
#pragma unroll
  for (int r = 0; r < 4; ++r) {
    const int uo = 16 * w + 4 * g + r;
    if (uo < M::W) {
#pragma unroll
      for (int nt = 0; nt < NT1; ++nt) {
        const int ui = 16 * nt + c;
        if (ui < M::W) W2[uo * M::W + ui] = G2[0][nt][r];
        else if (ui == M::W) b2[uo] = G2[0][nt][r];
      }
      if (c < M::IN0) W1[uo * M::IN0 + M::col0(c)] = G1[0][0][r];
      else if (c == M::IN0) b1[uo] = G1[0][0][r];
    }
    const int uh = 4 * g + r, ui = 16 * w + c;
    if (uh < C::H) {
      if (ui < M::W) W3[uh * M::W + ui] = G3[0][0][r];
      else if (ui == M::W) b3[uh] = G3[0][0][r];
    }
  }
  BWD_STAMP(3, wall_clock64());
}


template <class C, bool DROP, bool TAIL>
__global__ void __launch_bounds__(256, 2) k_ode_fwd_split(KArgs a) {
  __shared__ __attribute__((aligned(16))) float lds_raw[OdeFwdSplitLds<C>::FLOATS];
  const int n_items = TAIL ? a.B : a.n_obs;
  ode_fwd_split<C, DROP, TAIL, false>(a, (lfp)lds_raw, blockIdx.x, gridDim.x, 0, (n_items + 15) / 16);
}

template <class C, bool PLAN> struct OdeFwdMixedLds {
  static constexpr int OWN = OdeFwdSplitLds<C>::FLOATS;
  static constexpr int FLOATS = (PLAN && PLAN_LDS_INTS > OWN) ? PLAN_LDS_INTS : OWN;
};
template <class C, bool DROP, bool PLAN>
__device__ __forceinline__ void ode_fwd_mixed_body(const KArgs& a, lfp lds_raw, int bid, int nblocks) {
  const int n_tiles = (a.n_obs + 15) / 16, ns = a.n_split_fwd;
  const int T = (int)a.base_s[a.K + 2];
  const bool save = a.save_traj != 0;
  if (bid < ns) {
    if (save) ode_fwd_split<C, DROP, false, true>(a, lds_raw, bid, ns, 0, T);
    else ode_fwd_split<C, DROP, false, false>(a, lds_raw, bid, ns, 0, T);
  } else {
    const int wave = (bid - ns) * 4 + uniform(threadIdx.x >> 6);
    const int nw = (nblocks - ns) * 4;
    if (save) ode2_fwd_single<C, DROP, false, true>(a, threadIdx.x & 63, wave, nw, T, n_tiles);
    else ode2_fwd_single<C, DROP, false, false>(a, threadIdx.x & 63, wave, nw, T, n_tiles);
  }
}
template <class C, bool DROP>
__global__ void __launch_bounds__(256, 2) k_ode_fwd_mixed(KArgs a) {
  __shared__ __attribute__((aligned(16))) float lds_raw[OdeFwdMixedLds<C, false>::FLOATS];
  ode_fwd_mixed_body<C, DROP, false>(a, (lfp)lds_raw, blockIdx.x, gridDim.x);
}
template <class C, bool DROP>
__global__ void __launch_bounds__(256, 2) k_ode_fwd_mixed_plan(KArgs a, PlanJob job) {
  __shared__ __attribute__((aligned(16))) float lds_raw[OdeFwdMixedLds<C, true>::FLOATS];
  if ((int)blockIdx.x < job.P) {
    plan_grid_body(job, blockIdx.x, (int*)lds_raw);
    return;
  }
  ode_fwd_mixed_body<C, DROP, true>(a, (lfp)lds_raw, (int)blockIdx.x - job.P, (int)gridDim.x - job.P);
}
template <class C> struct OdeBwdMixedLds {
  static constexpr int A = OdeBwdActLds<C>::FLOATS, B = OdeBwdSplitLds<C>::FLOATS;
  static constexpr int FLOATS = A > B ? A : B;
};
template <class C, bool DROP>
__global__ void __launch_bounds__(256, 2) k_ode_bwd_mixed(KArgs a) {
  __shared__ __attribute__((aligned(16))) float lds_raw[OdeBwdMixedLds<C>::FLOATS];
  const int n_tiles = (a.n_obs + 15) / 16, ns = a.n_split_blocks;
  const int T = (int)a.base_s[a.K + 1];
#ifdef NJ_BWD_STAMPS
  BWD_STAMP(0, wall_clock64());
  BWD_STAMP(6, (unsigned long long)__builtin_amdgcn_s_getreg((31 << 11) | 4 ) |
                   ((unsigned long long)__builtin_amdgcn_s_getreg((31 << 11) | 20 ) << 32));
  BWD_STAMP(7, (unsigned long long)((int)blockIdx.x < ns ? 1 : 0) | ((unsigned long long)T << 8) |
                   ((unsigned long long)gridDim.x << 32));
#endif
  if ((int)blockIdx.x < ns) {
    ode3_bwd_split<C, DROP>(a, (lfp)lds_raw, blockIdx.x, ns, 0, T, blockIdx.x);
  } else {
    const int wave = ((int)blockIdx.x - ns) * 4 + uniform(threadIdx.x >> 6);
    ode3_bwd_single<C, DROP>(a, (lfp)lds_raw, wave, ((int)gridDim.x - ns) * 4, T, n_tiles, blockIdx.x);
  }
}

}
```

njode_amd/csrc/njode_ode2.h:

```cpp
#pragma once
#include "njode_mfma.h"
#include "njode_mfma_rows.h"

namespace njode {

constexpr float TANH_PRESCALE = 2.8853900817779268f;

template <class C> struct Ode2Scale {
  static constexpr float S = C::ACT == ACT_TANH ? TANH_PRESCALE : 1.0f;
};

template <class C> NJ_DEV float ode_frag_value(const float* __restrict__ P, int idx, float S, float ik) {
  using M = MF<C>;
  const int f = idx >> 6, l = idx & 63, g = l >> 4, c = l & 15;
  const float* Po = P + C::OFF_ODE;
  using NL = typename C::Ode;
  const float *W1 = Po + NL::woff(0), *b1 = Po + NL::boff(0), *W2 = Po + NL::woff(1),
              *b2 = Po + NL::boff(1), *W3 = Po + NL::woff(2), *b3 = Po + NL::boff(2);
  float v = 0.0f;
  if (f < M::F2) {
    const int mt = (f - M::F1) / M::Q0, q = (f - M::F1) % M::Q0;
    const int uo = row_unit(mt, c), ui = 4 * q + g;
    if (uo < M::W) v = S * (ui < M::IN0 ? W1[uo * M::IN0 + M::col0(ui)] : (ui == M::IN0 ? b1[uo] : 0.0f));
  } else if (f < M::F3) {
    const int mt = (f - M::F2) / M::Q1, q = (f - M::F2) % M::Q1;
    const int uo = row_unit(mt, c), ui = 4 * q + g;
    if (uo < M::W) v = ui < M::W ? S * ik * W2[uo * M::W + ui] : (ui == M::W ? S * b2[uo] : 0.0f);
  } else if (f < M::NFWD) {
    const int mt = (f - M::F3) / M::Q1, q = (f - M::F3) % M::Q1;
    const int uo = row_unit(mt, c), ui = 4 * q + g;
    if (uo < M::H) v = ui < M::W ? ik * W3[uo * M::W + ui] : (ui == M::W ? b3[uo] : 0.0f);
  } else if (f < M::B2) {
    const int mt = (f - M::B3) / M::QH, q = (f - M::B3) % M::QH;
    const int ui = row_unit(mt, c), uo = 4 * q + g;
    if (ui < M::W && uo < M::H) v = ik * W3[uo * M::W + ui];
  } else if (f < M::B1) {
    const int mt = (f - M::B2) / M::QW, q = (f - M::B2) % M::QW;
    const int ui = row_unit(mt, c), uo = 4 * q + g;
    if (ui < M::W && uo < M::W) v = ik * W2[uo * M::W + ui];
  } else {
    const int mt = (f - M::B1) / M::QW, q = (f - M::B1) % M::QW;
    const int u = row_unit(mt, c), uo = 4 * q + g;
    if (u < M::IN0 && uo < M::W) v = W1[uo * M::IN0 + M::col0(u)];
  }
  return v;
}
template <class C>
__global__ void k_pack_frags2(const float* __restrict__ P, float* __restrict__ frag, float ik) {
  const int idx = blockIdx.x * blockDim.x + threadIdx.x;
  if (idx >= MF<C>::NALL * 64) return;
  frag[idx] = ode_frag_value<C>(P, idx, Ode2Scale<C>::S, ik);
}
template <class C>
__global__ void k_pack_frags12(const float* __restrict__ P, float* __restrict__ frag,
                               float* __restrict__ frag2, float ik) {
  constexpr int N = MF<C>::NALL * 64;
  const int idx = blockIdx.x * blockDim.x + threadIdx.x;
  if (idx >= 2 * N) return;
  if (idx < N) frag[idx] = ode_frag_value<C>(P, idx, 1.0f, 1.0f);
  else frag2[idx - N] = ode_frag_value<C>(P, idx - N, Ode2Scale<C>::S, ik);
}

template <int ACT> NJ_DEV float act2_f(float zs) {
  if constexpr (ACT == ACT_TANH) {
    const float e = __builtin_amdgcn_exp2f(zs);
    return fmaf(__builtin_amdgcn_rcpf(e + 1.0f), -2.0f, 1.0f);
  } else {
    return fmaxf(zs, 0.0f);
  }
}


template <class C, int U> constexpr bool in0_var() {
  return U < C::H + C::D + 2 + (C::CURT ? 1 : 0);
}
template <class C> struct In0Const {
  float v[MF<C>::Q0];
  NJ_DEV void init(int g) {
    const float z[C::D] = {};
#pragma unroll
    for (int q = 0; q < MF<C>::Q0; ++q) v[q] = 0.0f;
    init_q<0>(g, z);
  }
  template <int Q> NJ_DEV void init_q(int g, const float (&z)[C::D]) {
    if constexpr (Q < MF<C>::Q0) {
      const float e0 = in0_var<C, 4 * Q + 0>() ? 0.0f : in0_unit<C, 4 * Q + 0>(0.0f, z, 0.0f, 0.0f);
      const float e1 = in0_var<C, 4 * Q + 1>() ? 0.0f : in0_unit<C, 4 * Q + 1>(0.0f, z, 0.0f, 0.0f);
      const float e2 = in0_var<C, 4 * Q + 2>() ? 0.0f : in0_unit<C, 4 * Q + 2>(0.0f, z, 0.0f, 0.0f);
      const float e3 = in0_var<C, 4 * Q + 3>() ? 0.0f : in0_unit<C, 4 * Q + 3>(0.0f, z, 0.0f, 0.0f);
      float x = g == 0 ? e0 : (g == 1 ? e1 : (g == 2 ? e2 : e3));
      asm volatile("" : "+v"(x));
      v[Q] = x;
      init_q<Q + 1>(g, z);
    }
  }
};
template <class C, int Q>
NJ_DEV void in0_fill_c(float (&b0)[MF<C>::Q0], const float (&h)[MF<C>::QH], const float (&tx)[C::D],
                       float tau, float tdiff, int g, const In0Const<C>& K) {
  if constexpr (Q < MF<C>::Q0) {
    float th = 0.0f;
    if constexpr (4 * Q < C::H) th = tanh_f(h[Q]);
    float x = K.v[Q];
    if constexpr (in0_var<C, 4 * Q + 3>()) x = g == 3 ? in0_unit<C, 4 * Q + 3>(th, tx, tau, tdiff) : x;
    if constexpr (in0_var<C, 4 * Q + 2>()) x = g == 2 ? in0_unit<C, 4 * Q + 2>(th, tx, tau, tdiff) : x;
    if constexpr (in0_var<C, 4 * Q + 1>()) x = g == 1 ? in0_unit<C, 4 * Q + 1>(th, tx, tau, tdiff) : x;
    if constexpr (in0_var<C, 4 * Q + 0>()) x = g == 0 ? in0_unit<C, 4 * Q + 0>(th, tx, tau, tdiff) : x;
    b0[Q] = x;
    in0_fill_c<C, Q + 1>(b0, h, tx, tau, tdiff, g, K);
  }
}

template <class C> struct StepRec {
  using M = MF<C>;
  static constexpr int Q1 = M::Q1, QH = M::QH;
  static constexpr int NF = Q1 / 4, L1 = Q1 % 4;
  static constexpr int NT = L1 + QH, NTQ = NT / 4, NTS = NT % 4;
  static constexpr int TAILQ = NF * 256;
  static constexpr int TAILS = (NF + NTQ) * 256;
  static constexpr int GA = TAILS + NTS * 64;
  static constexpr int B1S = GA + NF * 256;
  static constexpr int FLOATS = B1S + L1 * 64;
  static constexpr int PER_CHAIN = FLOATS / 16;
  static constexpr int WT = NF < 3 ? NF : 3;
  static_assert(FLOATS == (2 * Q1 + QH) * 64, "step record: every register exactly once");
};
template <class C> NJ_DEV float* rec_block(const float* act, long long b16, int tile) {
  return (float*)act + (size_t)(b16 + 16 * (long long)tile) * StepRec<C>::PER_CHAIN;
}
NJ_DEV void quad_store(float* p, float x, float y, float z, float w) {
  const f32x4 v = {x, y, z, w};
  *(f32x4*)p = v;
}
template <class C, int I>
NJ_DEV float rec_tail_get(const float (&a2)[MF<C>::Q1], const float (&h)[MF<C>::QH]) {
  using R = StepRec<C>;
  if constexpr (I < R::L1) return a2[4 * R::NF + I];
  else if constexpr (I < R::NT) return h[I - R::L1];
  else return 0.0f;
}
template <class C, int I>
NJ_DEV void rec_tail_put(float v, float (&a2)[MF<C>::Q1], float (&h)[MF<C>::QH]) {
  using R = StepRec<C>;
  if constexpr (I < R::L1) a2[4 * R::NF + I] = v;
  else if constexpr (I < R::NT) h[I - R::L1] = v;
}
template <class C, int K = 0>
NJ_DEV void rec_tail_store(float* blk, int lane, const float (&a2)[MF<C>::Q1], const float (&h)[MF<C>::QH]) {
  using R = StepRec<C>;
  if constexpr (K < R::NTQ) {
    quad_store(blk + R::TAILQ + K * 256 + lane * 4, rec_tail_get<C, 4 * K>(a2, h),
               rec_tail_get<C, 4 * K + 1>(a2, h), rec_tail_get<C, 4 * K + 2>(a2, h),
               rec_tail_get<C, 4 * K + 3>(a2, h));
    rec_tail_store<C, K + 1>(blk, lane, a2, h);
  } else if constexpr (K < R::NTQ + R::NTS) {
    blk[R::TAILS + (K - R::NTQ) * 64 + lane] = rec_tail_get<C, 4 * R::NTQ + (K - R::NTQ)>(a2, h);
    rec_tail_store<C, K + 1>(blk, lane, a2, h);
  }
}
template <class C, int K = 0>
NJ_DEV void rec_tail_load(const float* blk, int lane, float (&a2)[MF<C>::Q1], float (&h)[MF<C>::QH]) {
  using R = StepRec<C>;
  if constexpr (K < R::NTQ) {
    const f32x4 v = *(const f32x4*)(blk + R::TAILQ + K * 256 + lane * 4);
    rec_tail_put<C, 4 * K>(v[0], a2, h);
    rec_tail_put<C, 4 * K + 1>(v[1], a2, h);
    rec_tail_put<C, 4 * K + 2>(v[2], a2, h);
    rec_tail_put<C, 4 * K + 3>(v[3], a2, h);
    rec_tail_load<C, K + 1>(blk, lane, a2, h);
  } else if constexpr (K < R::NTQ + R::NTS) {
    rec_tail_put<C, 4 * R::NTQ + (K - R::NTQ)>(blk[R::TAILS + (K - R::NTQ) * 64 + lane], a2, h);
    rec_tail_load<C, K + 1>(blk, lane, a2, h);
  }
}
template <class C>
NJ_DEV void rec_store_A(float* blk, int lane, const float (&a2)[MF<C>::Q1], const float (&h)[MF<C>::QH]) {
  using R = StepRec<C>;
#pragma unroll
  for (int k = 0; k < R::NF; ++k)
    quad_store(blk + k * 256 + lane * 4, a2[4 * k], a2[4 * k + 1], a2[4 * k + 2], a2[4 * k + 3]);
  rec_tail_store<C>(blk, lane, a2, h);
}
template <class C>
NJ_DEV void rec_store_B(float* blk, int lane, const float (&a1)[MF<C>::Q1]) {
  using R = StepRec<C>;
#pragma unroll
  for (int k = 0; k < R::NF; ++k)
    quad_store(blk + R::GA + k * 256 + lane * 4, a1[4 * k], a1[4 * k + 1], a1[4 * k + 2], a1[4 * k + 3]);
#pragma unroll
  for (int i = 0; i < R::L1; ++i) blk[R::B1S + i * 64 + lane] = a1[4 * R::NF + i];
}
template <class C>
NJ_DEV void rec_load_A(const float* blk, int lane, float (&a2)[MF<C>::Q1], float (&h)[MF<C>::QH]) {
  using R = StepRec<C>;
#pragma unroll
  for (int k = 0; k < R::NF; ++k) {
    const f32x4 v = *(const f32x4*)(blk + k * 256 + lane * 4);
    a2[4 * k] = v[0]; a2[4 * k + 1] = v[1]; a2[4 * k + 2] = v[2]; a2[4 * k + 3] = v[3];
  }
  rec_tail_load<C>(blk, lane, a2, h);
}
template <class C>
NJ_DEV void rec_load_B(const float* blk, int lane, float (&a1)[MF<C>::Q1]) {
  using R = StepRec<C>;
#pragma unroll
  for (int k = 0; k < R::NF; ++k) {
    const f32x4 v = *(const f32x4*)(blk + R::GA + k * 256 + lane * 4);
    a1[4 * k] = v[0]; a1[4 * k + 1] = v[1]; a1[4 * k + 2] = v[2]; a1[4 * k + 3] = v[3];
  }
#pragma unroll
  for (int i = 0; i < R::L1; ++i) a1[4 * R::NF + i] = blk[R::B1S + i * 64 + lane];
}
NJ_DEV int uniform(int v) { return __builtin_amdgcn_readfirstlane(v); }
NJ_DEV void vm_drain() { __builtin_amdgcn_s_waitcnt(0x0F70); }
typedef const long long __attribute__((address_space(4))) * cllp;
NJ_DEV long long sload_ll(const long long* p, int i) { return ((cllp)(unsigned long long)p)[i]; }

template <int ACT, bool DROP> NJ_DEV float dact_stored(float av) {
  const float d = dact_f<ACT>(av);
  if constexpr (DROP) return __float_as_uint(av) == 0x80000000u ? 0.0f : d;
  else return d;
}

NJ_DEV uint32_t xs32(uint32_t& s) {
  s ^= s << 13; s ^= s >> 17; s ^= s << 5;
  return s;
}

template <class C, bool DROP, int MT0>
NJ_DEV void hidden_pair(const f32x4& t0, const f32x4& t1, float (&av)[MF<C>::Q1], uint32_t& s,
                        uint32_t thr16, int g) {
  constexpr int Q1 = MF<C>::Q1;
#pragma unroll
  for (int r = 0; r < 8; r += 2) {
    const int q = 4 * MT0 + r;
    if (q < Q1) {
      float v0 = act2_f<C::ACT>(r < 4 ? t0[r & 3] : t1[r & 3]);
      float v1 = q + 1 < Q1 ? act2_f<C::ACT>(r + 1 < 4 ? t0[(r + 1) & 3] : t1[(r + 1) & 3]) : 0.0f;
      if constexpr (DROP) {
        const uint32_t w = xs32(s);
        v0 = (w & 0xffffu) >= thr16 ? v0 : -0.0f;
        v1 = (w >> 16) >= thr16 ? v1 : -0.0f;
      }
      av[q] = v0;
      if (q + 1 < Q1) av[q + 1] = v1;
    }
  }
  constexpr int QB = MF<C>::W / 4, GB = MF<C>::W % 4;
  if constexpr (QB >= 4 * MT0 && QB < 4 * MT0 + 8) av[QB] = g == GB ? 1.0f : av[QB];
}

template <int MT, int Q, int MT0, int ET = -1, int ER = 0>
NJ_DEV void mfma_pair(const float (&A)[MT][Q], const float (&bv)[Q], f32x4& t0, f32x4& t1, int g = 0) {
  const f32x4 z = {0.f, 0.f, 0.f, 0.f};
  t0 = z;
  t1 = z;
#pragma unroll
  for (int q = 0; q < Q; ++q) {
    if constexpr (MT0 == ET) t0 = mfma1(A[MT0][q], bv[q], t0);
    else t0 = mfma4(A[MT0][q], bv[q], t0);
    if constexpr (MT0 + 1 < MT) {
      if constexpr (MT0 + 1 == ET) t1 = mfma1(A[MT0 + 1][q], bv[q], t1);
      else t1 = mfma4(A[MT0 + 1][q], bv[q], t1);
    }
  }
  if constexpr (MT0 == ET) t0 = edge_tile<ER>(t0, g);
  if constexpr (MT0 + 1 == ET && MT0 + 1 < MT) t1 = edge_tile<ER>(t1, g);
}

template <class C> struct Ode2FwdFrags {
  using M = MF<C>;
  float A1[M::MT1][M::Q0], A2[M::MT1][M::Q1], A3[M::MTH][M::Q1];
  NJ_DEV void load(const float* frag, int lane) {
#pragma unroll
    for (int mt = 0; mt < M::MT1; ++mt) {
      const int l = mt == EdgeRows<M::W>::TILE ? edge_lane(lane) : lane;
#pragma unroll
      for (int q = 0; q < M::Q0; ++q) A1[mt][q] = frag[(M::F1 + mt * M::Q0 + q) * 64 + l];
#pragma unroll
      for (int q = 0; q < M::Q1; ++q) A2[mt][q] = frag[(M::F2 + mt * M::Q1 + q) * 64 + l];
    }
#pragma unroll
    for (int mt = 0; mt < M::MTH; ++mt)
#pragma unroll
      for (int q = 0; q < M::Q1; ++q) A3[mt][q] = frag[(M::F3 + mt * M::Q1 + q) * 64 + lane];
  }
};

template <class C, bool DROP, int QIN, int MT0 = 0>
NJ_DEV void hidden_layer2(const float (&A)[MF<C>::MT1][QIN], const float (&bv)[QIN],
                          float (&av)[MF<C>::Q1], uint32_t& st, uint32_t thr16, int g) {
  if constexpr (MT0 < MF<C>::MT1) {
    f32x4 t0, t1;
    mfma_pair<MF<C>::MT1, QIN, MT0, EdgeRows<MF<C>::W>::TILE, EdgeRows<MF<C>::W>::R>(A, bv, t0, t1, g);
    hidden_pair<C, DROP, MT0>(t0, t1, av, st, thr16, g);
    hidden_layer2<C, DROP, QIN, MT0 + 2>(A, bv, av, st, thr16, g);
  }
}

template <class C>
NJ_DEV void out_layer2(const float (&A3)[MF<C>::MTH][MF<C>::Q1], const float (&a2)[MF<C>::Q1],
                       f32x4 (&f)[MF<C>::MTH]) {
  using M = MF<C>;
  const f32x4 z = {0.f, 0.f, 0.f, 0.f};
#pragma unroll
  for (int mt = 0; mt < M::MTH; ++mt) {
    f32x4 e = z, o = z;
#pragma unroll
    for (int q = 0; q < M::Q1; q += 2) {
      e = mfma4(A3[mt][q], a2[q], e);
      if (q + 1 < M::Q1) o = mfma4(A3[mt][q + 1], a2[q + 1], o);
    }
    f[mt] = e + o;
  }
}

template <class C, bool DROP, bool TAIL, bool SAVE>
NJ_DEV void ode2_fwd_single(const KArgs& a, int lane, int wave, int n_waves, int tile0, int tile1) {
  static_assert(!(TAIL && SAVE), "tail items are never checkpointed");
  using M = MF<C>;
  const int g = lane >> 4, c = lane & 15;
  Ode2FwdFrags<C> F;
  F.load(a.frag2, lane);
  In0Const<C> K0;
  K0.init(g);

  const int n_items = TAIL ? a.B : a.n_obs;
  const int n_tiles = tile1 - tile0;
  float* const trash = a.trash + lane * C::H;
  for (int round = 0; round * n_waves < n_tiles; ++round) {
    const int rel = snake_tile(round, wave, n_waves);
    if (rel >= n_tiles) continue;
    const int tile = tile0 + rel;
    const int j = tile * 16 + c;
    const bool valid = j < n_items;
    Item<C> it;
    it.template load<TAIL>(a, j, valid);
    float h[M::QH];
    const float* h0 = it.h0(a);
#pragma unroll
    for (int q = 0; q < M::QH; ++q) {
      const int u = 4 * q + g;
      h[q] = u < C::H ? h0[u < C::H ? u : 0] : 0.0f;
    }
    const int nmax = uniform(wave_max(it.n));
    float dt_r = 0.0f, t_r = 0.0f;
    long long b16_n = 0;
    if (nmax > 0) {
      const int k0 = it.n > 0 ? it.kbeg : 0;
      dt_r = a.step_dt[k0];
      t_r = a.step_t[k0];
      b16_n = SAVE ? sload_ll(a.base16_s, 0) : 0;
    }
    if constexpr (SAVE) {
      if (a.item_pack) {
        if (g == 0) it.store_pack(a.item_pack, j);
        const long long bl = sload_ll(a.base16_s, nmax > 0 ? nmax - 1 : 0);
        if (lane == 0) a.tile_last[tile] = bl;
      }
    }
    vm_drain();
    for (int s = 0; s < nmax; ++s) {
      const bool active = s < it.n;
      const int k = active ? it.kbeg + s : 0;
      const float dt = active ? dt_r : 0.0f, t = t_r;
      const long long b16 = b16_n;
      {
        const int sn = s + 1 < nmax ? s + 1 : s;
        const int kn = sn < it.n ? it.kbeg + sn : 0;
// ... 87 lines not shown
                       f32x4 (&G1)[MF<C>::MT1][(MF<C>::IN0 + 1 + 15) / 16], int slab_row) {
  using M = MF<C>;
  using NL = typename C::Ode;
  using E2 = OdeG2<C>;
  constexpr int NT1 = (M::W + 1 + 15) / 16, NT0 = (M::IN0 + 1 + 15) / 16;
  const int lane = threadIdx.x & 63, wv = threadIdx.x >> 6, g = lane >> 4, c = lane & 15;
  if constexpr (E2::ER != 0) {
    GM[0] += GM[1];
    GN[0] += GN[1];
  }
  constexpr int NG = M::MTH * NT1 + E2::MT * E2::NT + (E2::ER ? 2 : 0) + M::MT1 * NT0;
  static_assert(3 * NG * 64 * 4 <= OdeBwdActLds<C>::FLOATS, "tile reduction does not fit the LDS");
  __syncthreads();
  f32x4 __attribute__((address_space(3)))* red = (f32x4 __attribute__((address_space(3)))*)lds_raw;
  auto for_tiles = [&](auto f) {
    int i = 0;
#pragma unroll
    for (int mt = 0; mt < M::MTH; ++mt)
#pragma unroll
      for (int nt = 0; nt < NT1; ++nt) f(G3[mt][nt], i++);
#pragma unroll
    for (int mt = 0; mt < E2::MT; ++mt)
#pragma unroll
      for (int nt = 0; nt < E2::NT; ++nt) f(G2[mt][nt], i++);
    if constexpr (E2::ER != 0) {
      f(GM[0], i++);
      f(GN[0], i++);
    }
#pragma unroll
    for (int mt = 0; mt < M::MT1; ++mt)
#pragma unroll
      for (int nt = 0; nt < NT0; ++nt) f(G1[mt][nt], i++);
  };
  if (wv > 0) for_tiles([&](f32x4& t, int i) { red[((wv - 1) * NG + i) * 64 + lane] = t; });
  __syncthreads();
  if (wv != 0) return;
  for_tiles([&](f32x4& t, int i) {
    t += red[(0 * NG + i) * 64 + lane];
    t += red[(1 * NG + i) * 64 + lane];
    t += red[(2 * NG + i) * 64 + lane];
  });
  const float ik = DROP ? a.dc.inv_keep : 1.0f;
  float* slab = a.slab + (size_t)slab_row * C::P + C::OFF_ODE;
  float *W1 = slab + NL::woff(0), *b1 = slab + NL::boff(0), *W2 = slab + NL::woff(1),
        *b2 = slab + NL::boff(1), *W3 = slab + NL::woff(2), *b3 = slab + NL::boff(2);
#pragma unroll
  for (int mt = 0; mt < E2::MT; ++mt)
#pragma unroll
    for (int r = 0; r < 4; ++r) {
      const int uo = 16 * mt + 4 * g + r;
      if (uo < M::W) {
#pragma unroll
        for (int nt = 0; nt < E2::NT; ++nt) {
          const int ui = 16 * nt + c;
          if (ui < M::W) W2[uo * M::W + ui] = ik * G2[mt][nt][r];
          else if (ui == M::W) b2[uo] = G2[mt][nt][r];
        }
      }
    }
  if constexpr (E2::ER != 0) {
#pragma unroll
    for (int i = 0; i < E2::ER; ++i) {
      const int uo = 16 * E2::ET + i;
      if (lane < M::W) W2[uo * M::W + lane] = ik * GM[0][i];
      else if (lane == M::W) b2[uo] = GM[0][i];
    }
    if (lane < 16 * E2::ET) {
#pragma unroll
      for (int i = 0; i < 4; ++i) {
        const int ui = 16 * E2::ET + i;
        if (ui < M::W) W2[lane * M::W + ui] = ik * GN[0][i];
        else if (ui == M::W) b2[lane] = GN[0][i];
      }
    }
  }
#pragma unroll
  for (int mt = 0; mt < M::MT1; ++mt)
#pragma unroll
    for (int r = 0; r < 4; ++r) {
      const int uo = 16 * mt + 4 * g + r;
      if (uo < M::W) {
#pragma unroll
        for (int nt = 0; nt < NT0; ++nt) {
          const int ui = 16 * nt + c;
          if (ui < M::IN0) W1[uo * M::IN0 + M::col0(ui)] = G1[mt][nt][r];
          else if (ui == M::IN0) b1[uo] = G1[mt][nt][r];
        }
      }
    }
#pragma unroll
  for (int mt = 0; mt < M::MTH; ++mt)
#pragma unroll
    for (int r = 0; r < 4; ++r) {
      const int uo = 16 * mt + 4 * g + r;
      if (uo < C::H) {
#pragma unroll
        for (int nt = 0; nt < NT1; ++nt) {
          const int ui = 16 * nt + c;
          if (ui < M::W) W3[uo * M::W + ui] = ik * G3[mt][nt][r];
          else if (ui == M::W) b3[uo] = G3[mt][nt][r];
        }
      }
    }
}

#ifdef NJ_BWD_STAMPS
__device__ unsigned long long g_bwd_stamps[8192 * 16];
#define BWD_STAMP(slot, val) \
  do { if ((threadIdx.x & 63) == 0) g_bwd_stamps[(size_t)(blockIdx.x * 4 + (threadIdx.x >> 6)) * 16 + (slot)] = (val); } while (0)
#else
#define BWD_STAMP(slot, val) do {} while (0)
#endif

template <class C, bool DROP>
NJ_DEV void ode3_bwd_single(const KArgs& a, lfp lds_raw, int wave, int n_waves, int tile0, int tile1,
                            int slab_row) {
  using M = MF<C>;
  using NL = typename C::Ode;
  using FR = OdeLdsFragsT<C>;
  constexpr int NT1 = (M::W + 1 + 15) / 16;
  constexpr int NT0 = (M::IN0 + 1 + 15) / 16;
  const int lane = threadIdx.x & 63, wv = threadIdx.x >> 6, g = lane >> 4, c = lane & 15;
  using IL = BwdIL;
  lfp img_d = lds_raw + wv * 2 * IL::FLOATS, img_a = img_d + IL::FLOATS;
  lfp fimg = lds_raw + 4 * 2 * IL::FLOATS;
  FR::stage(fimg, a.frag2, threadIdx.x, 256);
  for (int i = threadIdx.x; i < 4 * 2 * IL::FLOATS; i += 256) lds_raw[i] = 0.0f;
  __syncthreads();
  FR F;
  F.init(fimg, lane);
  In0Const<C> K0;
  K0.init(g);

  using E2 = OdeG2<C>;
  constexpr int ET = E2::ER ? E2::ET : -1, ER = E2::ER;
  const int de = edge_lane(lane) - lane;
  f32x4 G3[M::MTH][NT1], G2[E2::MT][E2::NT], GM[2], GN[2], G1[M::MT1][NT0];
  const f32x4 zero4 = {0.f, 0.f, 0.f, 0.f};
  GM[0] = GM[1] = GN[0] = GN[1] = zero4;
#pragma unroll
  for (int i = 0; i < M::MTH; ++i)
#pragma unroll
    for (int n = 0; n < NT1; ++n) G3[i][n] = zero4;
#pragma unroll
  for (int i = 0; i < E2::MT; ++i)
#pragma unroll
    for (int n = 0; n < E2::NT; ++n) G2[i][n] = zero4;
#pragma unroll
  for (int i = 0; i < M::MT1; ++i) {
#pragma unroll
    for (int n = 0; n < NT0; ++n) G1[i][n] = zero4;
  }
  float* const trash = a.trash + threadIdx.x * C::H;
  const int n_tiles = tile1 - tile0;
  BWD_STAMP(1, wall_clock64());
  int n_done = 0, n_steps_done = 0;
#ifdef NJ_BWD_STAMPS
  unsigned long long t_pro = 0, t_loop = 0;
#endif
  for (int round = 0; round * n_waves < n_tiles; ++round) {
#ifdef NJ_BWD_STAMPS
    const unsigned long long tt0 = wall_clock64();
#endif
    const int rel = snake_tile(round, wave, n_waves);
    if (rel >= n_tiles) continue;
    const int tile = tile0 + rel;
    const int j = tile * 16 + c;
    const bool valid = j < a.n_obs;
    Item<C> it;
    long long b16_last = 0;
    const bool packed = a.item_pack != nullptr;
    if (packed) {
      b16_last = sload_ll(a.tile_last, tile);
      it.load_pack(a.item_pack, j, valid);
    } else {
      it.template load<false>(a, j, valid);
    }
    float lam[M::QH];
#pragma unroll
    for (int q = 0; q < M::QH; ++q) {
      const int u = 4 * q + g;
      const float v = a.lam_end[(size_t)it.r * C::H + (u < C::H ? u : 0)];
      lam[q] = (valid && u < C::H) ? v : 0.0f;
    }
    const int nmax = BWD_ABL(64) ? 0 : uniform(wave_max(it.n));
    ++n_done;
    n_steps_done += nmax;
    auto load_sched = [&](int s, float& dtr, float& tr) {
      const int kk = s < it.n ? it.kbeg + s : 0;
      dtr = a.step_dt[kk];
      tr = a.step_t[kk];
    };
    float h[M::QH], a1[M::Q1], a2[M::Q1], dt_r = 0.0f, t_r = 0.0f;
#pragma unroll
    for (int q = 0; q < M::QH; ++q) h[q] = 0.0f;
#pragma unroll
    for (int q = 0; q < M::Q1; ++q) { a1[q] = 0.0f; a2[q] = 0.0f; }
    if (nmax > 0) {
      const float* blk = rec_block<C>(a.act, packed ? b16_last : sload_ll(a.base16_s, nmax - 1), tile);
      load_sched(nmax - 1, dt_r, t_r);
      rec_load_A<C>(blk, lane, a2, h);
      rec_load_B<C>(blk, lane, a1);
    }
#ifdef NJ_BWD_STAMPS
    vm_drain();
    const unsigned long long tt1 = wall_clock64();
    t_pro += tt1 - tt0;
#endif
    for (int s = nmax - 1; s >= 0; --s) {
      const float dt = s < it.n ? dt_r : 0.0f, t = t_r;
      const int sp = s > 0 ? s - 1 : 0;
      const float* blkp = rec_block<C>(a.act, sload_ll(a.base16_s, sp), tile);
      float b0[M::Q0];
      in0_fill_c<C, 0>(b0, h, it.tx, it.tau, t - it.tau, g, K0);
      if (!BWD_ABL(8)) load_sched(sp, dt_r, t_r);
      F.begin();

      float d3[M::QH];
#pragma unroll
      for (int q = 0; q < M::QH; ++q) d3[q] = dt * lam[q];
      if (!BWD_ABL(16)) {
        img_write<M::QH, IL>(img_d, d3, g, c);
        img_write<M::Q1, IL>(img_a, a2, g, c);
      }
      if (!BWD_ABL(4)) wave_lds_sync();
      if (!BWD_ABL(1)) dw_accumulate<M::MTH, NT1, IL>(img_d, img_a, G3, g, c);
      f32x4 acc[M::MT1];
#pragma unroll
      for (int mt = 0; mt < M::MT1; ++mt) acc[mt] = zero4;
      if (!BWD_ABL(2)) {
#pragma unroll
        for (int q = 0; q < M::QH; ++q)
#pragma unroll
          for (int mt = 0; mt < M::MT1; ++mt)
            acc[mt] = mt == ET ? mfma1(F.e3(q, de), d3[q], acc[mt]) : mfma4(F.b3(mt, q), d3[q], acc[mt]);
        if constexpr (ER != 0) acc[ET] = edge_tile<ER>(acc[ET], g);
      } else {
#pragma unroll
        for (int mt = 0; mt < M::MT1; ++mt) acc[mt][0] = d3[0];
      }
      float d2[M::QW];
#pragma unroll
      for (int q = 0; q < M::QW; ++q)
        d2[q] = acc[q / 4][q % 4] * (BWD_ABL(32) ? 1.0f : dact_stored<C::ACT, DROP>(a2[q]));
      if (!BWD_ABL(8)) rec_load_A<C>(blkp, lane, a2, h);
      if (!BWD_ABL(4)) wave_lds_sync();

      if (!BWD_ABL(16)) {
        img_write<M::QW, IL>(img_d, d2, g, c);
        img_write<M::Q1, IL>(img_a, a1, g, c);
      }
      if (!BWD_ABL(4)) wave_lds_sync();
      if (!BWD_ABL(1)) {
        if constexpr (ER != 0) dw_accumulate_edge<E2::MT, IL>(img_d, img_a, G2, GM, GN, lane, g, c);
        else dw_accumulate<E2::MT, E2::NT, IL>(img_d, img_a, G2, g, c);
      }
#pragma unroll
      for (int mt = 0; mt < M::MT1; ++mt) acc[mt] = zero4;
      if (!BWD_ABL(2)) {
#pragma unroll
        for (int q = 0; q < M::QW; ++q)
#pragma unroll
          for (int mt = 0; mt < M::MT1; ++mt)
            acc[mt] = mt == ET ? mfma1(F.e2(q, de), d2[q], acc[mt]) : mfma4(F.b2(mt, q), d2[q], acc[mt]);
        if constexpr (ER != 0) acc[ET] = edge_tile<ER>(acc[ET], g);
      } else {
#pragma unroll
        for (int mt = 0; mt < M::MT1; ++mt) acc[mt][0] = d2[mt];
      }
      float d1[M::QW];
#pragma unroll
      for (int q = 0; q < M::QW; ++q)
        d1[q] = acc[q / 4][q % 4] * (BWD_ABL(32) ? 1.0f : dact_stored<C::ACT, DROP>(a1[q]));
      if (!BWD_ABL(8)) rec_load_B<C>(blkp, lane, a1);
      if (!BWD_ABL(4)) wave_lds_sync();

      if (!BWD_ABL(16)) {
        img_write<M::QW, IL>(img_d, d1, g, c);
        img_write<M::Q0, IL>(img_a, b0, g, c);
      }
      if (!BWD_ABL(4)) wave_lds_sync();
      if (!BWD_ABL(1)) dw_accumulate<M::MT1, NT0, IL>(img_d, img_a, G1, g, c);
      f32x4 acch[M::MTH];
#pragma unroll
      for (int mt = 0; mt < M::MTH; ++mt) {
        f32x4 e = zero4, o = zero4;
        if (!BWD_ABL(2)) {
#pragma unroll
          for (int q = 0; q < M::QW; q += 2) {
            e = mfma4(F.b1(mt, q), d1[q], e);
            if (q + 1 < M::QW) o = mfma4(F.b1(mt, q + 1), d1[q + 1], o);
          }
        } else {
          e[0] = d1[0];
        }
        acch[mt] = e + o;
      }
#pragma unroll
      for (int q = 0; q < M::QH; ++q) {
        const float th = b0[q];
        const float dth = (4 * q + g) < C::H ? 1.0f - th * th : 0.0f;
        lam[q] = fmaf(acch[q / 4][q % 4], dth, lam[q]);
      }
      if (!BWD_ABL(4)) wave_lds_sync();
    }
#ifdef NJ_BWD_STAMPS
    t_loop += wall_clock64() - tt1;
#endif
    float* out = valid ? a.lam_start + (size_t)it.r * C::H : trash;
#pragma unroll
    for (int q = 0; q < M::QH; ++q) {
      const int u = 4 * q + g;
      float* dst = u < C::H ? out + u : trash;
      *dst = lam[q];
    }
  }

#ifdef NJ_BWD_STAMPS
  BWD_STAMP(8, t_pro);
  BWD_STAMP(9, t_loop);
#endif
  BWD_STAMP(2, wall_clock64());
  BWD_STAMP(4, (unsigned long long)n_done);
  BWD_STAMP(5, (unsigned long long)n_steps_done);
  (void)n_done; (void)n_steps_done;
  if (BWD_ABL(128)) return;
  ode3_flush<C, DROP>(a, lds_raw, G3, G2, GM, GN, G1, slab_row);
  BWD_STAMP(3, wall_clock64());
}


}
```

njode_amd/csrc/njode_plan.h:

```cpp
#pragma once
#include <hip/hip_runtime.h>

namespace njode {

constexpr int PLAN_KEYS = 512;
constexpr int PLAN_TIMES = 1500;
constexpr int PLAN_THREADS = 256;
constexpr int PLAN_LDS_INTS = 4 * PLAN_KEYS + 96;
constexpr int PLAN_SCAN_CHUNKS = 32;
constexpr int SPLIT_KMAX = 4095;
struct SplitCfg { int on, ns[2], nw[2]; float r[2]; };

struct PlanJob {
  int P;
  int first_stage;
  int last_stage;
  int n, B, K, n_times;
  int cs_shift, cs_nwb;
  const int* sched_src;
  int* sched_dst;
  int sched_ints;
  const int* time_ptr;
  const int* k_jump;
  const int* obs_idx;
  int* t_of_row;
  int* dense;
  int* first_row;
  int* last_row;
  int* item_prev;
  int* item_next;
  int* item_kbeg;
  int* item_len;
  unsigned* sort_key;
  int* len_hist;
  int* cs_tab;
  int* order;
  long long* base_s;
  long long* base16_s;
  unsigned* sync;
  unsigned sync_base;
  unsigned* fail;
  unsigned long long* stamps;
  SplitCfg sc;
};

template <bool COH, class T> __device__ __forceinline__ T pld(const T* p) {
  if constexpr (COH) return __hip_atomic_load(p, __ATOMIC_RELAXED, __HIP_MEMORY_SCOPE_AGENT);
  else return *p;
}
template <bool COH, class T> __device__ __forceinline__ void pst(T* p, T v) {
  if constexpr (COH) __hip_atomic_store(p, v, __ATOMIC_RELAXED, __HIP_MEMORY_SCOPE_AGENT);
  else *p = v;
}
constexpr int PLAN_SPIN_MAX = 1 << 22;
__device__ inline void plan_sync(unsigned* ctr, unsigned base, int P, unsigned* fail) {
  if (P > 1) {
    asm volatile("s_waitcnt vmcnt(0)" ::: "memory");
    __syncthreads();
    if (threadIdx.x == 0) {
      __hip_atomic_fetch_add(ctr, 1u, __ATOMIC_RELAXED, __HIP_MEMORY_SCOPE_AGENT);
      int spins = 0;
      while ((int)(__hip_atomic_load(ctr, __ATOMIC_RELAXED, __HIP_MEMORY_SCOPE_AGENT) - base) < P) {
        if (++spins > PLAN_SPIN_MAX) {
          if (fail) __hip_atomic_store(fail, 1u, __ATOMIC_RELAXED, __HIP_MEMORY_SCOPE_AGENT);
          break;
        }
        __builtin_amdgcn_s_sleep(2);
      }
      asm volatile("s_waitcnt vmcnt(0)" ::: "memory");
    }
    __syncthreads();
  } else {
    __syncthreads();
  }
}

constexpr int traj_layout_lds_ints(int kmax, int nt) { return ((kmax + 2) & ~1) + 6 * (nt / 64); }
template <int NT, bool COH = false>
__device__ inline void traj_layout_body(const int* len_hist, int n_obs, int K, long long* base_s,
                                        long long* base16_s, const SplitCfg& sc, int* lds, bool lds_cnt) {
  constexpr int NWV = NT / 64;
  int* cnt = lds;
  long long* wsum = (long long*)(lds + ((K + 2) & ~1));
  float* best_c = (float*)(wsum + NWV);
  int* best_t = (int*)(best_c + 2 * NWV);
  const int tid = threadIdx.x;
  auto block_excl = [&](long long v, long long* total) -> long long {
    long long incl = v;
#pragma unroll
    for (int o = 1; o < 64; o <<= 1) {
      const long long up = __shfl_up(incl, o);
      if ((tid & 63) >= o) incl += up;
    }
    __syncthreads();
    if ((tid & 63) == 63) wsum[tid >> 6] = incl;
    __syncthreads();
    long long before = 0, all = 0;
    for (int i = 0; i < NWV; ++i) {
      if (i < (tid >> 6)) before += wsum[i];
      all += wsum[i];
    }
    if (total) *total = all;
    return before + incl - v;
  };
  if (lds_cnt) {
    const int ch = (K + 1 + NT - 1) / NT;
    for (int s = tid; s <= K; s += NT) cnt[s] = pld<COH>(len_hist + s);
    __syncthreads();
    {
      long long loc = 0;
      for (int q = 0; q < ch; ++q) {
        const int s = K - (tid * ch + q);
        if (s >= 0) loc += cnt[s];
      }
      long long run = block_excl(loc, nullptr);
      for (int q = 0; q < ch; ++q) {
        const int s = K - (tid * ch + q);
        if (s >= 0) {
          const int h = cnt[s];
          cnt[s] = (int)run;
          run += h;
        }
      }
    }
    __syncthreads();
    {
      long long loc = 0;
      for (int q = 0; q < ch; ++q) {
        const int s = tid * ch + q;
        if (s <= K) loc += cnt[s];
      }
      long long run = block_excl(loc, nullptr);
      for (int q = 0; q < ch; ++q) {
        const int s = tid * ch + q;
        if (s <= K) {
          base_s[s] = run;
          run += cnt[s];
        }
      }
    }
    __syncthreads();
    {
      long long loc = 0;
      for (int q = 0; q < ch; ++q) {
        const int s = tid * ch + q;
        if (s <= K) loc += (cnt[s] + 15) & ~15;
      }
      long long run = block_excl(loc, nullptr);
      for (int q = 0; q < ch; ++q) {
        const int s = tid * ch + q;
        if (s <= K) {
          base16_s[s] = run;
          run += (cnt[s] + 15) & ~15;
        }
      }
    }
    __syncthreads();
  } else if (tid == 0) {
    long long above = 0;
    for (int s = K; s >= 0; --s) {
      const long long h = len_hist[s];
      base_s[s] = above;
      above += h;
    }
// ... 324 lines not shown
```

njode_amd/csrc/njode_route.h:

```cpp
#pragma once
#include <algorithm>

#include "njode_env.h"
#include "njode_host.h"
#include "njode_hostlib.h"

namespace njode {

constexpr int SLAB_ROWS_MAX = 3072;
constexpr size_t DENSE_CELLS_MAX = (size_t)64 << 20;

struct Sizing {
  bool train, save;
  bool seg_any;
  bool seg_untailed;
  bool seg_items;
  bool chain;
  int q4_pt;
  size_t dense_cells;
  bool seg_bits;
  bool seg_act;
  bool pack;
  bool lock_act;
  bool lock_bits;
  bool delta, delta_seg;
  int n_waves;
  int n_waves_lock;
  int slab_rows;
};

inline Sizing size_call(const CfgOps& o, int B, int n_obs, int n_times, int K, int call_flags,
                        double rec_budget, const Env& e) {
  Sizing z;
  const bool want_path = (call_flags & NJODE_C_RETURN_PATH) != 0;
  const int steps = K > 0 ? K : 1;
  z.train = (call_flags & NJODE_C_TRAIN) != 0;
  z.save = (call_flags & NJODE_C_SAVE_BWD) != 0;
  z.seg_any = !(o.dims.flags & (NJODE_F_MASKED | NJODE_F_USE_RNN)) && (call_flags & NJODE_C_GET_LOSS) && !want_path;
  z.seg_untailed = z.seg_any && !((call_flags & NJODE_C_SCHED_KNOWN) && (call_flags & NJODE_C_SCHED_TAIL));
  const bool chain_rec_fit = !z.save || (double)B * steps * (CHAIN_ACT_FLOATS * 4.0 + 16.0) <= rec_budget;
  z.seg_items = o.seg_chain && e.ode == ODE_MFMA && !e.ode_one_wave && n_obs > 0 &&
                n_obs + B <= e.seg_chain_max && K <= SPLIT_KMAX && chain_rec_fit;
  z.chain = o.lock_chain && B <= e.chain_max && !(want_path && z.train) && chain_rec_fit;
  if (e.lock4_pt == 1 || e.lock4_pt == 2 || e.lock4_pt == 4 || e.lock4_pt == 8 || e.lock4_pt == 16) {
    z.q4_pt = e.lock4_pt;
  } else {
    z.q4_pt = 1;
    while (z.q4_pt < 16 && cdiv(B, z.q4_pt) > 256) z.q4_pt *= 2;
    if (o.lock_act_floats > 0 && z.save && !want_path) {
      const double per_tile = (double)steps * ((double)o.lock_act_floats * 4.0 + 256.0);
      while (z.q4_pt < 16 && (double)cdiv(B, z.q4_pt) * per_tile > rec_budget) z.q4_pt *= 2;
    }
  }
  const size_t cells = (size_t)(n_times > 0 ? n_times : 1) * (size_t)(B > 0 ? B : 1);
  z.dense_cells = (z.seg_any && n_obs > 0 && cells <= DENSE_CELLS_MAX) ? cells : 0;
  z.seg_bits = o.act_floats > 0 && z.seg_any && n_obs > 0 && z.train && (cdiv(n_obs, 16) <= 768 || z.seg_items);
  z.seg_act = z.save && o.act_floats > 0 && z.seg_untailed && n_obs > 0;
  z.pack = z.seg_act && e.item_pack;
  z.lock_act = z.save && (z.chain || (o.lock_act_floats > 0 && !want_path));
  z.lock_bits = z.train && (z.chain || z.lock_act);
  z.delta = z.save && e.chain_delta && (z.chain || (z.seg_act && z.seg_items)) &&
            (double)B * steps * (2.0 * CHAIN_ACT_FLOATS * 4.0 + 16.0) <= rec_budget;
  z.delta_seg = z.delta && o.dims.width < 64;
  const int row_tiles = cdiv(n_obs + B, 16) + 128;
  z.n_waves = std::max(4, (std::min(row_tiles, MAX_WAVES) + 3) & ~3);
  const long long w = ((long long)B * K / 16 + 7) / 8;
  z.n_waves_lock = ((int)std::min<long long>(1024, std::max<long long>(w, z.n_waves)) + 3) & ~3;
  z.slab_rows = std::max({std::min(row_tiles, SLAB_ROWS_MAX), z.n_waves, z.n_waves_lock, 576});
  return z;
}

enum LockKind { LOCK_VALU, LOCK_WAVE1, LOCK_TILE4, LOCK_CHAIN };
struct Route {
  Sizing size;
  bool drop;
  bool want_path, want_loss;
  bool seg;
  bool tails;
  int ode;
  bool seg_mfma;
  int lock_sweep, lock_fwd;
  int lock_fwd_kind, lock_bwd_kind;
  bool lock_bits_ahead;
  int chain_wpb;
  bool lock_mfma;
  int seg_ode;
  int ode_split;
  int seg_chain;
  int enc_blocks;
  bool tails_ride;
  bool seg_bits_ahead;
  bool side, tails_side;
  int defer_loss;
  int dw_enc_fused;
  int n_split_blocks, n_blocks_bwd, n_split_fwd, n_blocks_fwd;
  int dw_pair_blocks, dw_seg_blocks;
  bool chain_dw;
  bool dw_stored;
  bool hosts_plan;
  bool needs_PT;
};

inline int lock_kind(const CfgOps& o, const Sizing& z, const Env& e, bool mfma, bool want_path) {
  if (!mfma) return LOCK_VALU;
  if (z.chain) return LOCK_CHAIN;
  if (o.lock_act_floats > 0 && !want_path && e.lock4 && (!z.save || z.lock_act)) return LOCK_TILE4;
  return LOCK_WAVE1;
}

inline Route route_call(const CfgOps& o, const Sizing& z, int B, int n_obs, int K, int call_flags,
                        const Env& e, bool tail, bool drop, bool want_hT) {
  Route r;
  r.size = z;
  r.drop = drop;
  r.want_path = (call_flags & NJODE_C_RETURN_PATH) != 0;
  r.want_loss = (call_flags & NJODE_C_GET_LOSS) != 0;
  r.seg = z.seg_any && n_obs > 0 && !tail && !(call_flags & NJODE_C_GEN_LOCKSTEP);
  r.tails = r.seg && want_hT;
  r.ode = e.ode;
  r.seg_mfma = r.seg && r.ode == ODE_MFMA && o.seg_mfma;
  r.lock_sweep = !o.lock_sweep_mfma ? ODE_VALU
                 : (o.dims.flags & NJODE_F_MASKED) ? ODE_MFMA
                 : (r.ode == ODE_MFMA && !e.lock_sweep_valu) ? ODE_MFMA : ODE_VALU;
  r.lock_fwd = (z.lock_act || drop) ? r.lock_sweep : r.ode;
  r.lock_fwd_kind = lock_kind(o, z, e, r.lock_fwd == ODE_MFMA && o.lock_fwd_mfma, r.want_path);
  r.lock_bwd_kind = lock_kind(o, z, e, r.lock_sweep == ODE_MFMA, r.want_path);
  r.lock_bits_ahead = r.lock_fwd_kind == LOCK_TILE4 && drop && z.lock_bits && e.drop_bits_ahead;
  r.chain_wpb = 1;
  if (e.chain_wpb >= 1 && e.chain_wpb <= CHAIN_MAX_WAVES) r.chain_wpb = e.chain_wpb;
  else while (r.chain_wpb < CHAIN_MAX_WAVES && cdiv(B, r.chain_wpb) > 256) r.chain_wpb *= 2;
  r.lock_mfma = !r.seg && r.lock_sweep == ODE_MFMA;
  r.seg_ode = (r.ode == ODE_MFMA && !o.seg_mfma) ? ODE_VALU : r.ode;
  r.ode_split = (r.ode == ODE_MFMA && o.ode_split && !e.ode_one_wave && K <= SPLIT_KMAX) ? 1 : 0;
  r.defer_loss = !(z.save && r.seg_mfma) ? 0
                 : (call_flags & NJODE_C_LOSS_IN_BWD) ? 1 : (call_flags & NJODE_C_ROWS_IN_FWD) ? 2 : 0;
  const int n_tiles = cdiv(n_obs > 0 ? n_obs : 1, 16);
  if (n_tiles <= 384) {
    r.n_split_blocks = r.n_blocks_bwd = n_tiles;
  } else {
    const int tot_b = e.bwd_blocks > 0 ? e.bwd_blocks : 1024;
    r.n_split_blocks = e.split_bwd_blocks;
    int nsb = tot_b - e.split_bwd_blocks;
    if (nsb > cdiv(n_tiles, 4)) nsb = cdiv(n_tiles, 4);
    if (r.n_split_blocks + nsb > z.slab_rows) nsb = z.slab_rows - r.n_split_blocks;
    r.n_blocks_bwd = r.n_split_blocks + nsb;
  }
  if (n_tiles <= 768) {
    r.n_split_fwd = r.n_blocks_fwd = n_tiles;
  } else {
    r.n_split_fwd = e.split_fwd_blocks;
    int nsb = e.fwd_blocks - e.split_fwd_blocks;
    if (nsb > cdiv(n_tiles, 4)) nsb = cdiv(n_tiles, 4);
    r.n_blocks_fwd = r.n_split_fwd + nsb;
  }
  r.seg_chain = (r.seg_mfma && r.ode_split && z.seg_items) ? 1 : 0;
  r.enc_blocks = e.enc_blocks;
  r.tails_ride = r.tails && r.seg_chain;
  r.seg_bits_ahead = r.seg_mfma && drop && z.seg_bits &&
                     (r.seg_chain || (r.ode_split && e.drop_bits_ahead && r.n_split_fwd == r.n_blocks_fwd));
  r.side = r.tails_side = false;
  {
    const long long tiles = ((long long)B * (K > 0 ? K : 0) + 15) / 16, seg_tiles = ((long long)n_obs + B + 15) / 16;
    r.dw_pair_blocks = (int)std::min<long long>((tiles + 3) / 4, o.dims.hidden_size <= 16 ? 512 : 256);
    r.dw_seg_blocks = (int)std::min<long long>(std::max<long long>((seg_tiles + 3) / 4, 1), 64);
  }
  r.chain_dw = (z.chain || r.seg_chain) && z.delta && z.delta_seg;
  r.dw_stored = r.chain_dw && r.dw_pair_blocks > 0;
  r.dw_enc_fused = (e.dw_enc_fused && r.seg_chain && r.dw_stored) ? 1 : 0;
  r.hosts_plan = r.seg_mfma && r.ode_split;
  r.needs_PT = !(r.lock_mfma || r.seg_mfma);
  return r;
}

inline void route_side(Route& r, bool side) {
  r.side = side;
  r.tails_side = r.tails && side && !r.tails_ride;
  r.seg_bits_ahead = r.seg_bits_ahead && (r.seg_chain || !side);
}

inline bool route_admitted(const Route& r) {
  const Sizing& z = r.size;
  const bool chain = r.lock_fwd_kind == LOCK_CHAIN || r.lock_bwd_kind == LOCK_CHAIN;
  const bool tile4 = r.lock_fwd_kind == LOCK_TILE4 || r.lock_bwd_kind == LOCK_TILE4;
  return !(r.seg_chain && !z.seg_items) && !(chain && !z.chain) && !(tile4 && z.save && !z.lock_act) &&
         !(r.seg_bits_ahead && !z.seg_bits) && !(r.lock_bits_ahead && !z.lock_bits) &&
         !(r.lock_fwd_kind == LOCK_CHAIN && r.drop && !z.lock_bits);
}

struct SlabRows { int ode, enc, dec; };
inline SlabRows slab_rows_written(const Route& r) {
  const Sizing& z = r.size;
  const int rows = r.seg_mfma ? z.n_waves / 4 : z.n_waves;
  SlabRows s{!r.seg || r.seg_chain ? z.n_waves : r.ode_split ? r.n_blocks_bwd : rows, rows, rows};
  if (r.lock_mfma) s.ode = s.enc = s.dec = z.n_waves_lock;
  if (r.chain_dw) s.ode = r.dw_pair_blocks + r.dw_seg_blocks;
  return s;
}

}
```

Before: 23.80 million paths/s.

## Balance backward ODE tiles across workers with a cost-model deal built in forward

Adds a device-side 'deal' builder, hosted as one extra block in the forward mixed ODE kernel. It assigns backward tiles to split blocks and waves as linked lists, balancing estimated per-tile step cost instead of using a fixed snake order. The backward split and wave loops now walk these lists through a TileWalk helper that reads the next tile from scalar memory. The aim is to remove load imbalance in the backward pass, at the cost of an extra block, LDS pressure, some workspace, and a chained next-tile load per iteration.

```diff
diff --git a/include/njode_selftest.h b/include/njode_selftest.h
--- a/include/njode_selftest.h
+++ b/include/njode_selftest.h
@@ -43,6 +43,13 @@
 int njode_debug_plan_view(const NjodeDims* dims, int32_t batch_size, int32_t n_obs, int32_t n_times,
                           int32_t n_steps, int32_t call_flags, NjodePlanView* out);
 
+typedef struct NjodeDealView {
+  int64_t deal, base_s;
+  int32_t n_tiles, n_split_blocks, n_blocks_bwd, next_off;
+} NjodeDealView;
+int njode_debug_deal_view(const NjodeDims* dims, int32_t batch_size, int32_t n_obs, int32_t n_times,
+                          int32_t n_steps, int32_t call_flags, NjodeDealView* out);
+
 #ifdef __cplusplus
 }
 #endif
diff --git a/njode_amd/_lib.py b/njode_amd/_lib.py
--- a/njode_amd/_lib.py
+++ b/njode_amd/_lib.py
@@ -39,7 +39,8 @@
            'njode_f64_supported', 'njode_f64_workspace_bytes', 'njode_forward_f64', 'njode_backward_f64',
            'njode_gob_supported', 'njode_gob_param_count', 'njode_gob_workspace_bytes',
            'njode_gob_forward_f32', 'njode_gob_backward_f32',
-           'njode_selftest_dropout_words', 'njode_debug_plan_stamps', 'njode_debug_plan_view')
+           'njode_selftest_dropout_words', 'njode_debug_plan_stamps', 'njode_debug_plan_view',
+           'njode_debug_deal_view')
 ROWS_CLOSEST, ROWS_FIRST_NEAREST = 0, 1
 SDE_MODELS = {'BlackScholes': 0, 'OrnsteinUhlenbeck': 1, 'Heston': 2}
 SDE_MODELS_STAGED = dict(SDE_MODELS, HestonWOFeller=3)
diff --git a/njode_amd/csrc/njode_api.hip b/njode_amd/csrc/njode_api.hip
--- a/njode_amd/csrc/njode_api.hip
+++ b/njode_amd/csrc/njode_api.hip
@@ -425,6 +425,7 @@
   a.ode_split = r.ode_split, a.seg_chain = r.seg_chain;
   a.defer_loss = r.defer_loss;
   a.n_split_blocks = r.n_split_blocks, a.n_blocks_bwd = r.n_blocks_bwd;
+  a.bwd_deal = (r.bwd_deal && c.L.bwd_deal) ? (int*)(w + c.L.bwd_deal) : nullptr;
   a.n_split_fwd = r.n_split_fwd, a.n_blocks_fwd = r.n_blocks_fwd;
   a.dw_pair_blocks = r.dw_pair_blocks, a.dw_seg_blocks = r.dw_seg_blocks, a.dw_enc_fused = r.dw_enc_fused;
   return NJODE_OK;
@@ -474,6 +475,38 @@
 extern "C" int njode_plan_bytes(const NjodeDims* dims, int32_t batch_size, int32_t n_obs,
                                 int32_t n_times, int32_t n_steps, int32_t call_flags, size_t* out) {
   return size_query(dims, batch_size, n_obs, n_times, n_steps, call_flags, out, true);
+}
+
+extern "C" int njode_debug_deal_view(const NjodeDims* dims, int32_t batch_size, int32_t n_obs, int32_t n_times,
+                                     int32_t n_steps, int32_t call_flags, NjodeDealView* out) {
+  if (!dims || !out) return fail(NJODE_E_BADARG, "null argument");
+  memset(out, 0, sizeof(*out));
+  out->deal = out->base_s = -1;
+  if (!find_cfg(dims) || n_obs <= 0) return NJODE_OK;
+  alignas(256) static char anchor[256];
+  NjodeBatch b{};
+  b.batch_size = batch_size;
+  b.n_obs = n_obs;
+  b.start_X = b.X = b.M = (const float*)anchor;
+  b.obs_idx = b.n_obs_ot = (const int32_t*)anchor;
+  b.loss_batch_size = 1.0f;
+  NjodeSchedule s{};
+  s.n_steps = n_steps;
+  s.n_times = n_times;
+  s.step_dt = s.step_t = s.time_f32 = (const float*)anchor;
+  s.k_jump = s.time_ptr = (const int32_t*)anchor;
+  Call c;
+  const int flags = (call_flags & ~(NJODE_C_PLAN_READY | NJODE_C_PLAN_DEFER | NJODE_C_SCHED_TAIL)) | NJODE_C_SCHED_KNOWN;
+  if (int rc = prepare(c, dims, (const float*)anchor, &b, &s, flags, 0.5f, 0.0f, 0, anchor, (size_t)-1,
+                       false))
+    return rc;
+  out->deal = c.a.bwd_deal ? (int64_t)((const char*)c.a.bwd_deal - anchor) : -1;
+  out->base_s = (int64_t)((const char*)c.a.base_s - anchor);
+  out->n_tiles = cdiv(n_obs, 16);
+  out->n_split_blocks = c.a.n_split_blocks;
+  out->n_blocks_bwd = c.a.n_blocks_bwd;
+  out->next_off = DEAL_NEXT_OFF;
+  return NJODE_OK;
 }
 
 extern "C" int njode_debug_plan_view(const NjodeDims* dims, int32_t batch_size, int32_t n_obs, int32_t n_times,
diff --git a/njode_amd/csrc/njode_cfg.hip b/njode_amd/csrc/njode_cfg.hip
--- a/njode_amd/csrc/njode_cfg.hip
+++ b/njode_amd/csrc/njode_cfg.hip
@@ -180,12 +180,14 @@
       if (r.ode_split) {
         if constexpr (TAIL) {
           k_ode_fwd_split<CC, DROP, true><<<n_tiles < 1024 ? n_tiles : 1024, 256, 0, st>>>(a);
+        } else {
+          const int nd = (a.bwd_deal && a.save_traj) ? 1 : 0;
+          if (a.plan_job) {
+            const PlanJob job = *(const PlanJob*)a.plan_job;
+            k_ode_fwd_mixed_plan<CC, DROP><<<a.n_blocks_fwd + job.P + nd, 256, 0, st>>>(a, job);
+          }
+          else k_ode_fwd_mixed<CC, DROP><<<a.n_blocks_fwd + nd, 256, 0, st>>>(a);
         }
-        else if (a.plan_job) {
-          const PlanJob job = *(const PlanJob*)a.plan_job;
-          k_ode_fwd_mixed_plan<CC, DROP><<<a.n_blocks_fwd + job.P, 256, 0, st>>>(a, job);
-        }
-        else k_ode_fwd_mixed<CC, DROP><<<a.n_blocks_fwd, 256, 0, st>>>(a);
         return;
       }
     }
diff --git a/njode_amd/csrc/njode_deal.h b/njode_amd/csrc/njode_deal.h
--- /dev/null
+++ b/njode_amd/csrc/njode_deal.h
@@ -0,0 +1,335 @@
+#pragma once
+#include <hip/hip_runtime.h>
+
+#include "njode_plan.h"
+
+namespace njode {
+
+constexpr int DEAL_CLASSES = 4;
+constexpr int DEAL_THREADS = 256;
+constexpr int DEAL_WPT = DEAL_WORKERS_MAX / DEAL_THREADS;
+constexpr int DEAL_LDS_INTS = (DEAL_KMAX + 1) + 3 * DEAL_WORKERS_MAX + DEAL_RES_BLOCKS + 32;
+static_assert(3 * (DEAL_LDS_INTS * 4 + 1024) <= 160 * 1024 && DEAL_THREADS <= DEAL_RES_BLOCKS, "three hosting blocks per CU");
+
+struct DealJob {
+  const long long* base_s;
+  int n_obs, K, ns, nb;
+  int* out;
+};
+
+__device__ inline int deal_class_min(int c) { return c == 0 ? 9 : c == 1 ? 5 : c == 2 ? 3 : 1; }
+
+__device__ inline void deal_build(const DealJob& j, int* lds) {
+  constexpr int NT = DEAL_THREADS, NWV = NT / 64, WPT = DEAL_WPT;
+  const int tid = threadIdx.x;
+  const int K = j.K, ns = j.ns, nb = j.nb;
+  const int n = (j.n_obs + 15) / 16;
+  const int T = (int)j.base_s[K + 1];
+  const int nw = 4 * (nb - ns);
+  const int nres = nb < DEAL_RES_BLOCKS ? nb : DEAL_RES_BLOCKS;
+  const int nf = nb > nres ? 4 * (nres - ns) : nw;
+  const int n2 = (nw - nf) / 4;
+  int* cnt = lds;
+  int* cq = cnt + DEAL_KMAX + 1;
+  int* lload = cq + DEAL_WORKERS_MAX;
+  int* rstart = lload + DEAL_WORKERS_MAX;
+  int* ends = rstart + DEAL_WORKERS_MAX;
+  int* fs = ends;
+  long long* wsum = (long long*)(ends + DEAL_RES_BLOCKS);
+  long long* pbnd = wsum + NWV;
+  int* head = j.out;
+  int* next = j.out + DEAL_NEXT_OFF;
+
+  auto block_sum = [&](long long v) -> long long {
+#pragma unroll
+    for (int o = 32; o > 0; o >>= 1) v += __shfl_xor(v, o);
+    __syncthreads();
+    if ((tid & 63) == 0) wsum[tid >> 6] = v;
+    __syncthreads();
+    long long all = 0;
+    for (int i = 0; i < NWV; ++i) all += wsum[i];
+    return all;
+  };
+  auto block_excl = [&](long long v, long long* total) -> long long {
+    long long incl = v;
+#pragma unroll
+    for (int o = 1; o < 64; o <<= 1) {
+      const long long up = __shfl_up(incl, o);
+      if ((tid & 63) >= o) incl += up;
+    }
+    __syncthreads();
+    if ((tid & 63) == 63) wsum[tid >> 6] = incl;
+    __syncthreads();
+    long long before = 0, all = 0;
+    for (int i = 0; i < NWV; ++i) {
+      if (i < (tid >> 6)) before += wsum[i];
+      all += wsum[i];
+    }
+    if (total) *total = all;
+    return before + incl - v;
+  };
+
+  for (int s = tid; s <= K; s += NT) cnt[s] = s < K ? (int)(j.base_s[s + 1] - j.base_s[s]) : 0;
+  __syncthreads();
+  auto len = [&](int t) {
+    int a = 0, b = K + 1;
+    while (a < b) {
+      const int m = (a + b) >> 1;
+      if (cnt[m] > 16 * t) a = m + 1; else b = m;
+    }
+    return a;
+  };
+  auto c1 = [&](int l) { return DEAL_C1_STEP * l + DEAL_C1_TILE; };
+
+  for (int b = tid; b < ns; b += NT) {
+    int prev = -1, f = DEAL_BLOCK_OVH;
+    head[b] = -1;
+    for (int r = 0; r * ns < T; ++r) {
+      const int t = r * ns + ((r & 1) ? ns - 1 - b : b);
+      if (t >= T) continue;
+      if (prev < 0) head[b] = t; else next[prev] = t;
+      next[t] = -1;
+      prev = t;
+      f += DEAL_C4_STEP * len(t) + DEAL_C4_TILE;
+    }
+    ends[b] = f;
+  }
+  const int nhead = nw < n - T ? nw : n - T;
+  const int m0 = T + nhead;
+  int ld[WPT], gg[WPT], tl[WPT];
+#pragma unroll
+  for (int q = 0; q < WPT; ++q) {
+    const int u = tid * WPT + q;
+    const int t = u < nhead ? T + u : -1;
+    ld[q] = t >= 0 ? c1(len(t)) : 0;
+    gg[q] = 0;
+    tl[q] = t;
+    if (u < nw) {
+      head[ns + u] = t;
+      if (t >= 0) next[t] = -1;
+    }
+    lload[u] = ld[q];
+  }
+  __syncthreads();
+  if (m0 >= n) return;
+
+  const int chunk = (n - T + NT - 1) / NT;
+  const int lo = T + tid * chunk < n ? T + tid * chunk : n;
+  const int hi = lo + chunk < n ? lo + chunk : n;
+  int bnd[DEAL_CLASSES + 1];
+  bnd[0] = m0;
+#pragma unroll
+  for (int c = 0; c < DEAL_CLASSES; ++c) {
+    const int cm = deal_class_min(c) - 1;
+    int e = cm <= K ? (cnt[cm] + 15) / 16 : 0;
+    e = e < bnd[c] ? bnd[c] : e;
+    bnd[c + 1] = e > n ? n : e;
+  }
+  const int l_lo = lo < n ? len(lo) : 0;
+  long long mine = 0;
+  {
+    int lcur = l_lo;
+    for (int t = lo; t < hi; ++t) {
+      while (lcur > 0 && cnt[lcur - 1] <= 16 * t) --lcur;
+      mine += c1(lcur);
+    }
+  }
+  long long ctot_ll = 0;
+  const long long pre_lo = block_excl(mine, &ctot_ll);
+  {
+    int lcur = l_lo;
+    long long run = pre_lo;
+    for (int t = lo; t < hi; ++t) {
+      while (lcur > 0 && cnt[lcur - 1] <= 16 * t) --lcur;
+#pragma unroll
+      for (int c = 0; c <= DEAL_CLASSES; ++c)
+        if (bnd[c] == t) pbnd[c] = run;
+      run += c1(lcur);
+    }
+  }
+  if (tid == 0) {
+#pragma unroll
+    for (int c = 0; c <= DEAL_CLASSES; ++c)
+      if (bnd[c] == n) pbnd[c] = ctot_ll;
+  }
+  const int ctot = (int)ctot_ll;
+  long long sumF = 0;
+  for (int b = tid; b < ns; b += NT) sumF += ends[b];
+  sumF = block_sum(sumF);
+  const int big = 2 * (ctot + (int)sumF) + 64;
+
+  int A;
+  if (n2 > 0) {
+    const long long xhat = (ctot_ll + 4 * sumF + (long long)DEAL_BLOCK_OVH * nw + 4 * nres - 1) / (4 * nres);
+    A = (int)(xhat / 2) - DEAL_BLOCK_OVH;
+    A = A > 0 ? A : 0;
+  } else {
+    int a = 0, b = big;
+    while (b - a > 1) {
+      const int mid = (a + b) >> 1;
+      long long s = 0;
+#pragma unroll
+      for (int q = 0; q < WPT; ++q)
+        if (tid * WPT + q < nf) s += ld[q] > mid ? ld[q] : mid;
+      if (block_sum(s) >= ctot_ll) b = mid; else a = mid;
+    }
+    A = b;
+  }
+  long long gfirst = 0;
+#pragma unroll
+  for (int q = 0; q < WPT; ++q) {
+    const int u = tid * WPT + q;
+    if (u < nf) {
+      gg[q] = A > ld[q] ? A : ld[q];
+      gfirst += gg[q];
+    }
+  }
+#pragma unroll
+  for (int q = 0; q < WPT; q += 4) {
+    const int u = tid * WPT + q;
+    if (u < nf && n2 > 0) {
+      int e = gg[q];
+      e = gg[q + 1] > e ? gg[q + 1] : e;
+      e = gg[q + 2] > e ? gg[q + 2] : e;
+      e = gg[q + 3] > e ? gg[q + 3] : e;
+      ends[ns + u / 4] = DEAL_BLOCK_OVH + e;
+    }
+  }
+  gfirst = block_sum(gfirst);
+  if (n2 > 0) {
+    int* sorted = cq;
+    const int ne = ns + nf / 4;
+    for (int i = tid; i < ne; i += NT) {
+      const int v = ends[i];
+      int rank = 0;
+      for (int k = 0; k < ne; ++k) rank += (ends[k] < v || (ends[k] == v && k < i)) ? 1 : 0;
+      sorted[rank] = v;
+    }
+    __syncthreads();
+    int base2[WPT];
+#pragma unroll
+    for (int q = 0; q < WPT; ++q) {
+      const int u = tid * WPT + q;
+      base2[q] = (u >= nf && u < nw) ? sorted[(u - nf) / 4] + DEAL_BLOCK_OVH : 0;
+    }
+    const long long need = ctot_ll - gfirst;
+    int a = 0, b = big;
+    while (b - a > 1) {
+      const int mid = (a + b) >> 1;
+      long long s = 0;
+#pragma unroll
+      for (int q = 0; q < WPT; ++q) {
+        const int u = tid * WPT + q;
+        if (u >= nf && u < nw) s += mid - base2[q] > ld[q] ? mid - base2[q] : ld[q];
+      }
+      if (block_sum(s) >= need) b = mid; else a = mid;
+    }
+#pragma unroll
+    for (int q = 0; q < WPT; ++q) {
+      const int u = tid * WPT + q;
+      if (u >= nf && u < nw) gg[q] = b - base2[q] > ld[q] ? b - base2[q] : ld[q];
+    }
+  }
+  __syncthreads();
+
+  for (int c = 0; c < DEAL_CLASSES; ++c) {
+    const int ca = bnd[c], cb = bnd[c + 1];
+    if (cb == ca) continue;
+    const long long pa = pbnd[c], need = pbnd[c + 1] - pa;
+#pragma unroll
+    for (int q = 0; q < WPT; ++q) ld[q] = lload[tid * WPT + q];
+    int a = -big, b = big;
+    while (b - a > 1) {
+      const int mid = a + ((b - a) >> 1);
+      long long s = 0;
+#pragma unroll
+      for (int q = 0; q < WPT; ++q) {
+        const int room = gg[q] - ld[q] - mid;
+        if (tid * WPT + q < nw) s += room > 0 ? room : 0;
+      }
+      if (block_sum(s) >= need) a = mid; else b = mid;
+    }
+    long long qsum = 0;
+    int qq[WPT];
+#pragma unroll
+    for (int q = 0; q < WPT; ++q) {
+      const int room = gg[q] - ld[q] - a;
+      qq[q] = (tid * WPT + q < nw && room > 0) ? room : 0;
+      qsum += qq[q];
+    }
+    long long run = block_excl(qsum, nullptr);
+#pragma unroll
+    for (int q = 0; q < WPT; ++q) {
+      run += qq[q];
+      cq[tid * WPT + q] = (int)run;
+      rstart[tid * WPT + q] = -1;
+    }
+    __syncthreads();
+    auto owner_from = [&](int u, long long mid2) {
+      while (u < nw - 1 && 2ll * cq[u] <= mid2) ++u;
+      return u;
+    };
+    auto owner_search = [&](long long mid2) {
+      int x = 0, y = nw - 1;
+      while (x < y) {
+        const int m = (x + y) >> 1;
+        if (2ll * cq[m] > mid2) y = m; else x = m + 1;
+      }
+      return x;
+    };
+    const int t0 = lo > ca ? lo : ca, t1 = hi < cb ? hi : cb;
+    if (t0 < t1) {
+      int lcur = l_lo;
+      long long p = pre_lo;
+      for (int t = lo; t < t0; ++t) {
+        while (lcur > 0 && cnt[lcur - 1] <= 16 * t) --lcur;
+        p += c1(lcur);
+      }
+      int prev_own = -1;
+      if (t0 > ca) {
+        const int lp = len(t0 - 1);
+        prev_own = owner_search(2 * (p - c1(lp) - pa) + c1(lp));
+      }
+      int own = prev_own < 0 ? 0 : prev_own;
+      for (int t = t0; t < t1; ++t) {
+        while (lcur > 0 && cnt[lcur - 1] <= 16 * t) --lcur;
+        const int ct = c1(lcur);
+        const long long mid2 = 2 * (p - pa) + ct;
+        own = t == t0 ? owner_search(mid2) : owner_from(own, mid2);
+        if (own != prev_own) {
+          if (prev_own >= 0) next[t - 1] = -1;
+          rstart[own] = t;
+        } else {
+          next[t - 1] = t;
+        }
+        atomicAdd(&lload[own], ct);
+        prev_own = own;
+        p += ct;
+      }
+      if (t1 == cb) next[cb - 1] = -1;
+    }
+    __syncthreads();
+    {
+      int first = -1;
+#pragma unroll
+      for (int q = WPT - 1; q >= 0; --q) first = rstart[tid * WPT + q] >= 0 ? rstart[tid * WPT + q] : first;
+      fs[tid] = first;
+      __syncthreads();
+      int following = cb;
+      for (int k = tid + 1; k < NT; ++k)
+        if (fs[k] >= 0) { following = fs[k]; break; }
+#pragma unroll
+      for (int q = WPT - 1; q >= 0; --q) {
+        const int u = tid * WPT + q, rs = rstart[u];
+        if (u < nw && rs >= 0) {
+          if (tl[q] >= 0) next[tl[q]] = rs; else head[ns + u] = rs;
+          tl[q] = following - 1;
+          following = rs;
+        }
+      }
+    }
+    __syncthreads();
+  }
+}
+
+}
diff --git a/njode_amd/csrc/njode_env.h b/njode_amd/csrc/njode_env.h
--- a/njode_amd/csrc/njode_env.h
+++ b/njode_amd/csrc/njode_env.h
@@ -7,7 +7,7 @@
 constexpr int ODE_MFMA = 0, ODE_VALU = 1;
 
 struct Env {
-  bool lock4, drop_bits_ahead, generic, ode_one_wave, sort_merge, sort_rocprim, item_pack, chain_delta, lock_sweep_valu,
+  bool lock4, drop_bits_ahead, generic, ode_one_wave, sort_merge, sort_rocprim, item_pack, bwd_deal, chain_delta, lock_sweep_valu,
       dw_enc_fused, tail_sort_rocprim, validate, plan_sort, plan_grid, plan_stamps, plan_stream, plan_grid_tail;
   int lock4_pt, chain_max, seg_chain_max, ode, split_bwd_blocks, split_fwd_blocks, bwd_blocks, fwd_blocks,
       plan_blocks, cs_shift, plan_inline_max, plan_inline_blocks, enc_blocks, chain_wpb,
@@ -38,6 +38,7 @@
   e.sort_merge = is(sort, "merge");
   e.sort_rocprim = is(sort, "rocprim");
   e.item_pack = not_off("NJODE_ITEM_PACK");
+  e.bwd_deal = not_off("NJODE_BWD_DEAL");
   e.chain_delta = not_off("NJODE_CHAIN_DELTA");
   e.split_r_bwd = (float)real("NJODE_SPLIT_R_BWD", 2.25);
   e.split_r_fwd = (float)real("NJODE_SPLIT_R_FWD", 2.0);
diff --git a/njode_amd/csrc/njode_kernels.h b/njode_amd/csrc/njode_kernels.h
--- a/njode_amd/csrc/njode_kernels.h
+++ b/njode_amd/csrc/njode_kernels.h
@@ -114,6 +114,7 @@
   float* cseg;
   float* item_pack;
   long long* tile_last;
+  int* bwd_deal;
   int dw_pair_blocks, dw_seg_blocks;
   int dw_enc_fused;
   DropCtx dc;
diff --git a/njode_amd/csrc/njode_layout.h b/njode_amd/csrc/njode_layout.h
--- a/njode_amd/csrc/njode_layout.h
+++ b/njode_amd/csrc/njode_layout.h
@@ -14,7 +14,7 @@
   size_t len_hist = 0, dense = 0;
   size_t sched, PT, frag, trash, t_of_row, iota, path_sorted, row_by_path, first3, item4, sort_key,
       key_sorted, order, tail4, base_s, h0row, h0start, h_end, lam_end, g_h0, lam_start, loss_terms,
-      traj, slab, red_partial, sum_partial, sort_tmp, lk_lam, lk_src, lk_rows, lk_hstart, base16, act, dbits, dbits_row, lk_act, lk_jact, lk_delta, lk_seg, item_pack, tile_last, vflag, cs_small, plan_end;
+      traj, slab, red_partial, sum_partial, sort_tmp, lk_lam, lk_src, lk_rows, lk_hstart, base16, act, dbits, dbits_row, lk_act, lk_jact, lk_delta, lk_seg, item_pack, tile_last, bwd_deal, vflag, cs_small, plan_end;
   size_t sort_tmp_bytes = 0;
 };
 
@@ -75,6 +75,7 @@
     L.item_pack = L.take((size_t)cdiv((int)nr, 16) * 16 * packf * 4);
     L.tile_last = L.take((size_t)cdiv((int)nr, 16) * 8);
   }
+  if (z.deal) L.bwd_deal = L.take(deal_region_ints(cdiv((int)nr, 16)) * 4);
   if (z.chain) {
     L.lk_act = L.take((size_t)B * steps * CHAIN_ACT_FLOATS * 4);
     L.lk_jact = L.take(nr * (size_t)CHAIN_JACT_FLOATS * 4);
diff --git a/njode_amd/csrc/njode_mfma_split.h b/njode_amd/csrc/njode_mfma_split.h
--- a/njode_amd/csrc/njode_mfma_split.h
+++ b/njode_amd/csrc/njode_mfma_split.h
@@ -2,6 +2,7 @@
 #include "njode_mfma.h"
 #include "njode_ode2.h"
 #include "njode_plan.h"
+#include "njode_deal.h"
 
 namespace njode {
 
@@ -533,13 +534,13 @@
   const f32x4 z = {0.f, 0.f, 0.f, 0.f};
   f32x4 G3[1][1] = {{z}}, G2[1][NT1] = {{z, z, z, z}}, G1[1][1] = {{z}};
   float* const trash = a.trash + lane * C::H;
-  const int n_tiles = tile1 - tile0;
   BWD_STAMP(1, wall_clock64());
   int n_done = 0, n_steps_done = 0;
-  for (int round = 0; round * n_workers < n_tiles; ++round) {
-    const int rel = snake_tile(round, worker, n_workers);
-    if (rel >= n_tiles) continue;
-    const int tile = tile0 + rel;
+  TileWalk tw;
+  tw.begin(a.bwd_deal, worker, worker, n_workers, tile0, tile1);
+  while (tw.more()) {
+    const int tile = tw.tile;
+    tw.peek();
     const int j = tile * 16 + c;
     const bool valid = j < a.n_obs;
     Item<C> it;
@@ -637,6 +638,7 @@
         *dst = lam[q];
       }
     }
+    tw.advance();
   }
 
   BWD_STAMP(2, wall_clock64());
@@ -678,8 +680,16 @@
 
 template <class C, bool PLAN> struct OdeFwdMixedLds {
   static constexpr int OWN = OdeFwdSplitLds<C>::FLOATS;
-  static constexpr int FLOATS = (PLAN && PLAN_LDS_INTS > OWN) ? PLAN_LDS_INTS : OWN;
+  static constexpr int HOSTED = (PLAN && PLAN_LDS_INTS > DEAL_LDS_INTS) ? PLAN_LDS_INTS : DEAL_LDS_INTS;
+  static constexpr int FLOATS = HOSTED > OWN ? HOSTED : OWN;
 };
+NJ_DEV bool fwd_hosts_deal(const KArgs& a) { return a.bwd_deal != nullptr && a.save_traj != 0; }
+NJ_DEV void fwd_deal_block(const KArgs& a, lfp lds_raw) {
+  DealJob j;
+  j.base_s = a.base_s, j.n_obs = a.n_obs, j.K = a.K, j.ns = a.n_split_blocks, j.nb = a.n_blocks_bwd;
+  j.out = a.bwd_deal;
+  deal_build(j, (int*)lds_raw);
+}
 template <class C, bool DROP, bool PLAN>
 __device__ __forceinline__ void ode_fwd_mixed_body(const KArgs& a, lfp lds_raw, int bid, int nblocks) {
   const int n_tiles = (a.n_obs + 15) / 16, ns = a.n_split_fwd;
@@ -698,7 +708,12 @@
 template <class C, bool DROP>
 __global__ void __launch_bounds__(256, 2) k_ode_fwd_mixed(KArgs a) {
   __shared__ __attribute__((aligned(16))) float lds_raw[OdeFwdMixedLds<C, false>::FLOATS];
-  ode_fwd_mixed_body<C, DROP, false>(a, (lfp)lds_raw, blockIdx.x, gridDim.x);
+  const int nd = fwd_hosts_deal(a) ? 1 : 0;
+  if (nd && blockIdx.x == 0) {
+    fwd_deal_block(a, (lfp)lds_raw);
+    return;
+  }
+  ode_fwd_mixed_body<C, DROP, false>(a, (lfp)lds_raw, (int)blockIdx.x - nd, (int)gridDim.x - nd);
 }
 template <class C, bool DROP>
 __global__ void __launch_bounds__(256, 2) k_ode_fwd_mixed_plan(KArgs a, PlanJob job) {
@@ -707,7 +722,12 @@
     plan_grid_body(job, blockIdx.x, (int*)lds_raw);
     return;
   }
-  ode_fwd_mixed_body<C, DROP, true>(a, (lfp)lds_raw, (int)blockIdx.x - job.P, (int)gridDim.x - job.P);
+  const int nd = fwd_hosts_deal(a) ? 1 : 0;
+  if (nd && (int)blockIdx.x == job.P) {
+    fwd_deal_block(a, (lfp)lds_raw);
+    return;
+  }
+  ode_fwd_mixed_body<C, DROP, true>(a, (lfp)lds_raw, (int)blockIdx.x - job.P - nd, (int)gridDim.x - job.P - nd);
 }
 template <class C> struct OdeBwdMixedLds {
   static constexpr int A = OdeBwdActLds<C>::FLOATS, B = OdeBwdSplitLds<C>::FLOATS;
diff --git a/njode_amd/csrc/njode_ode2.h b/njode_amd/csrc/njode_ode2.h
--- a/njode_amd/csrc/njode_ode2.h
+++ b/njode_amd/csrc/njode_ode2.h
@@ -1,6 +1,7 @@
 #pragma once
 #include "njode_mfma.h"
 #include "njode_mfma_rows.h"
+#include "njode_plan.h"
 
 namespace njode {
 
@@ -215,6 +216,24 @@
 NJ_DEV void vm_drain() { __builtin_amdgcn_s_waitcnt(0x0F70); }
 typedef const long long __attribute__((address_space(4))) * cllp;
 NJ_DEV long long sload_ll(const long long* p, int i) { return ((cllp)(unsigned long long)p)[i]; }
+typedef const int __attribute__((address_space(4))) * cip;
+NJ_DEV int sload_i(const int* p, int i) { return ((cip)(unsigned long long)p)[i]; }
+
+struct TileWalk {
+  const int* deal;
+  int worker, n_workers, tile0, tile1, round, left, tile, nxt;
+  NJ_DEV void begin(const int* deal_, int slot, int worker_, int n_workers_, int tile0_, int tile1_) {
+    deal = deal_, worker = worker_, n_workers = n_workers_, tile0 = tile0_, tile1 = tile1_;
+    round = 0, left = tile1 - tile0, nxt = -1;
+    tile = deal ? sload_i(deal, slot) : tile0 + snake_tile(0, worker, n_workers);
+  }
+  NJ_DEV bool more() const { return tile >= tile0 && tile < tile1 && left > 0; }
+  NJ_DEV void peek() { if (deal) nxt = sload_i(deal + DEAL_NEXT_OFF, tile); }
+  NJ_DEV void advance() {
+    ++round, --left;
+    tile = deal ? nxt : tile0 + snake_tile(round, worker, n_workers);
+  }
+};
 
 template <int ACT, bool DROP> NJ_DEV float dact_stored(float av) {
   const float d = dact_f<ACT>(av);
@@ -608,19 +627,19 @@
     for (int n = 0; n < NT0; ++n) G1[i][n] = zero4;
   }
   float* const trash = a.trash + threadIdx.x * C::H;
-  const int n_tiles = tile1 - tile0;
   BWD_STAMP(1, wall_clock64());
   int n_done = 0, n_steps_done = 0;
 #ifdef NJ_BWD_STAMPS
   unsigned long long t_pro = 0, t_loop = 0;
 #endif
-  for (int round = 0; round * n_waves < n_tiles; ++round) {
+  TileWalk tw;
+  tw.begin(a.bwd_deal, a.n_split_blocks + wave, wave, n_waves, tile0, tile1);
+  while (tw.more()) {
 #ifdef NJ_BWD_STAMPS
     const unsigned long long tt0 = wall_clock64();
 #endif
-    const int rel = snake_tile(round, wave, n_waves);
-    if (rel >= n_tiles) continue;
-    const int tile = tile0 + rel;
+    const int tile = tw.tile;
+    tw.peek();
     const int j = tile * 16 + c;
     const bool valid = j < a.n_obs;
     Item<C> it;
@@ -770,6 +789,7 @@
       float* dst = u < C::H ? out + u : trash;
       *dst = lam[q];
     }
+    tw.advance();
   }
 
 #ifdef NJ_BWD_STAMPS
diff --git a/njode_amd/csrc/njode_plan.h b/njode_amd/csrc/njode_plan.h
--- a/njode_amd/csrc/njode_plan.h
+++ b/njode_amd/csrc/njode_plan.h
@@ -10,6 +10,19 @@
 constexpr int PLAN_SCAN_CHUNKS = 32;
 constexpr int SPLIT_KMAX = 4095;
 struct SplitCfg { int on, ns[2], nw[2]; float r[2]; };
+constexpr int DEAL_KMAX = 511;
+constexpr int DEAL_WORKERS_MAX = 4096;
+constexpr int DEAL_BLOCKS_MAX = 1024;
+constexpr int DEAL_RES_BLOCKS = 512;
+constexpr int DEAL_NEXT_OFF = DEAL_BLOCKS_MAX + DEAL_WORKERS_MAX;
+constexpr long long DEAL_COST_MAX = 1ll << 27;
+constexpr int DEAL_C1_STEP = 4, DEAL_C1_TILE = 3, DEAL_C4_STEP = 2, DEAL_C4_TILE = 2, DEAL_BLOCK_OVH = 5;
+inline long long deal_cost_bound(int B, int n_tiles, int K) {
+  return DEAL_C1_STEP * ((long long)K + (long long)B * K / 16 + 1) + (long long)DEAL_C1_TILE * n_tiles;
+}
+inline size_t deal_region_ints(int n_tiles) {
+  return (size_t)DEAL_NEXT_OFF + (size_t)((n_tiles + 15) & ~15);
+}
 
 struct PlanJob {
   int P;
diff --git a/njode_amd/csrc/njode_route.h b/njode_amd/csrc/njode_route.h
--- a/njode_amd/csrc/njode_route.h
+++ b/njode_amd/csrc/njode_route.h
@@ -21,6 +21,7 @@
   bool seg_bits;
   bool seg_act;
   bool pack;
+  bool deal;
   bool lock_act;
   bool lock_bits;
   bool delta, delta_seg;
@@ -57,6 +58,7 @@
   z.seg_bits = o.act_floats > 0 && z.seg_any && n_obs > 0 && z.train && (cdiv(n_obs, 16) <= 768 || z.seg_items);
   z.seg_act = z.save && o.act_floats > 0 && z.seg_untailed && n_obs > 0;
   z.pack = z.seg_act && e.item_pack;
+  z.deal = z.seg_act && e.bwd_deal;
   z.lock_act = z.save && (z.chain || (o.lock_act_floats > 0 && !want_path));
   z.lock_bits = z.train && (z.chain || z.lock_act);
   z.delta = z.save && e.chain_delta && (z.chain || (z.seg_act && z.seg_items)) &&
@@ -97,6 +99,7 @@
   int dw_pair_blocks, dw_seg_blocks;
   bool chain_dw;
   bool dw_stored;
+  bool bwd_deal;
   bool hosts_plan;
   bool needs_PT;
 };
@@ -154,6 +157,10 @@
     r.n_blocks_fwd = r.n_split_fwd + nsb;
   }
   r.seg_chain = (r.seg_mfma && r.ode_split && z.seg_items) ? 1 : 0;
+  r.bwd_deal = z.deal && r.seg_mfma && r.ode_split && !r.seg_chain && n_tiles > 384 && K <= DEAL_KMAX &&
+               r.n_blocks_bwd <= DEAL_BLOCKS_MAX && r.n_split_blocks < std::min(r.n_blocks_bwd, DEAL_RES_BLOCKS) &&
+               4 * (r.n_blocks_bwd - r.n_split_blocks) <= DEAL_WORKERS_MAX &&
+               deal_cost_bound(B, n_tiles, K) <= DEAL_COST_MAX;
   r.enc_blocks = e.enc_blocks;
   r.tails_ride = r.tails && r.seg_chain;
   r.seg_bits_ahead = r.seg_mfma && drop && z.seg_bits &&
```

Result: slower. 20.79 million paths/s (-12.6%).
